# bsxfun/pffdtd

Measured on AMD Instinct MI355X. Metric: Gvoxel-updates/s, higher is better.
Workload: dtype f32; 1 GPU; shoebox 1024^3 7-pt Cartesian fp32, Mb=11 freq-dependent walls (BASELINE.json configs[3]); Nb=12423680, Nbl=6205736, Nba=6254648, numerics=cpu-exact, parallelism=1 GPU, air_variant=0

## Files before the change

include/pffdtd_hip.h:

```cpp
#ifndef PFFDTD_HIP_H
#define PFFDTD_HIP_H

#include <stdint.h>
#include <stddef.h>

#ifdef __cplusplus
extern "C" {
#endif

#define PF_MMB 12
#define PF_MNM 64

typedef struct pf_matquad_f32 { float  b, bd, bDh, bFh; } pf_matquad_f32;
typedef struct pf_matquad_f64 { double b, bd, bDh, bFh; } pf_matquad_f64;

typedef struct pf_simdata {
   int64_t  *bn_ixyz;
   int64_t  *bnl_ixyz;
   int64_t  *bna_ixyz;
   int8_t   *Q_bna;
   int64_t  *in_ixyz;
   int64_t  *out_ixyz;
   int64_t  *out_reorder;
   uint16_t *adj_bn;
   void     *ssaf_bnl;
   uint8_t  *bn_mask;
   int8_t   *mat_bnl;
   int8_t   *K_bn;
   double   *in_sigs;
   double   *u_out;
   int64_t   Ns, Nr, Nt, Npts, Nx, Ny, Nz, Nb, Nbl, Nba;
   double    l, l2;
   int8_t    fcc_flag;
   int8_t    NN;
   int8_t    Nm;
   int8_t   *Mb;
   void     *mat_quads;
   void     *mat_beta;
   double    infac;
   double    sl2, lo2, a2, a1;
   int32_t   real_bytes;
} pf_simdata;

typedef enum pf_status {
   PF_OK = 0,
   PF_ERR_ARG = 1,
   PF_ERR_HIP = 2,
   PF_ERR_NODEV = 3,
   PF_ERR_STATE = 4
} pf_status;

#define PF_NUM_CPU_EXACT       0
#define PF_NUM_GPU_SAFEGUARDED 2

typedef struct pf_opts {
   int32_t device;
   int32_t numerics;
   int32_t slab_first;
   int32_t slab_last;
   int32_t readout_chunk;
   int32_t air_variant;
   int32_t air_chunk;
   int32_t timing;
   void   *ext_u0;
   void   *ext_u1;
   int32_t x_global0;
   int32_t layout;
   int32_t energy;
   int32_t multi_flags;
   int32_t transport;
   int32_t verify_exchange;
   int32_t only_slab;
   double  wall_scale;
} pf_opts;

#define PF_LAYOUT_AUTO      0
#define PF_LAYOUT_EXCHANGED 1
#define PF_LAYOUT_FILE      2

#define PF_TRANSPORT_AUTO 0
#define PF_TRANSPORT_PEER 1
#define PF_TRANSPORT_RCCL 2
#define PF_TRANSPORT_HOST 3

#define PF_MULTI_EVEN_SPLIT  1
#define PF_MULTI_ONE_THREAD  2
#define PF_MULTI_NO_PAIRS    4
#define PF_MULTI_FORCE_PAIRS 8
#define PF_MULTI_CUT_Z      16
#define PF_MULTI_CUT_X      32
#define PF_MULTI_MEASURE_WEIGHTS 128
#define PF_MULTI_NO_TRIPLES 64

typedef struct pf_timing {
   double  air_ms_total;
   int64_t air_launches;
   double  step_ms_total;
   int64_t steps;
   double  tb2_ms_total;
   int64_t tb2_launches;
   int64_t tb2_cells;
   double  tune_ms[3];
   int64_t air_path;
   int64_t tb2_lw;
   int64_t tb2_dirty_tiles;
   int64_t place_candidates;
   double  place_ms[3];
   int64_t wall_blocks[2];
   int64_t tb_steps_per_pass;
   int64_t wall_bricks;
   int64_t wall_three_steps;
   int64_t wall_profile;
} pf_timing;

typedef struct pf_engine pf_engine;

const char *pf_last_error(void);
const char *pf_version(void);
int         pf_device_count(void);
size_t      pf_grid_bytes(int64_t Nx, int64_t Ny, int64_t Nz, int32_t real_bytes);
int64_t     pf_grid_pitch(int64_t Nz, int32_t real_bytes);
void        pf_opts_default(pf_opts *o);

double      pf_run_sim(pf_simdata *sd);
double      pf_run_sim_devices(pf_simdata *sd, int32_t nslabs, const int32_t *devices, const pf_opts *base);
int         pf_slab_partition(const pf_simdata *sd, int32_t nslabs, int32_t even_split, int64_t *cuts);
int         pf_slab_partition_w(const pf_simdata *sd, int32_t nslabs, int32_t even_split, double wall_scale, int64_t *cuts);
int         pf_slab_partition_axis(const pf_simdata *sd, int32_t nslabs, int32_t even_split, double wall_scale, int32_t along_z, int64_t *cuts);
double      pf_slab_wall_scale(pf_simdata *sd, int32_t nslabs, int32_t device, const pf_opts *base);

typedef struct pf_multi pf_multi;
typedef struct pf_multi_info {
   int32_t nslabs;
   int32_t transport;
   int32_t rccl_self;
   int32_t exchange_verified;
   int64_t exchanges_checked;
   int32_t exchange_nonzero;
   int32_t cut_along_z;
   int64_t plane_bytes;
   double  last_run_seconds;
   char    transport_name[64];
   char    transport_note[256];
   double  wall_scale;
   int32_t wall_measured;
} pf_multi_info;
int  pf_multi_create(pf_simdata *sd, int32_t nslabs, const int32_t *devices, const pf_opts *base, pf_multi **out);
int  pf_multi_run(pf_multi *m, int64_t n0, int64_t nsteps);
int  pf_multi_get_info(pf_multi *m, pf_multi_info *info);
int  pf_multi_get_slab(pf_multi *m, int32_t g, int64_t *x0, int64_t *x1, int32_t *device, int32_t *paired, pf_engine **engine);
void pf_multi_destroy(pf_multi *m);

typedef struct pf_rccl_comm pf_rccl_comm;
int  pf_rccl_unique_id(void *id128);
int  pf_rccl_comm_create(const void *id128, int32_t nranks, int32_t rank, int32_t device, pf_rccl_comm **out);
int  pf_rccl_exchange(pf_rccl_comm *c, pf_engine *e, int32_t peer_lo, int32_t peer_hi);
void pf_rccl_comm_destroy(pf_rccl_comm *c);

int  pf_engine_create(const pf_simdata *sd, const pf_opts *opts, pf_engine **out);
void pf_engine_destroy(pf_engine *e);
int  pf_engine_run(pf_engine *e, int64_t n0, int64_t nsteps);
int  pf_engine_step_begin(pf_engine *e, int64_t n);
int  pf_engine_halo_ptrs(pf_engine *e, void **send_lo, void **send_hi, void **recv_lo, void **recv_hi,
                         size_t *plane_bytes);
int  pf_engine_step_end(pf_engine *e, int64_t n);
int  pf_engine_set_spares(pf_engine *e, void *grid2, void *grid3);
int  pf_engine_place_grids(pf_engine *e, void *const *pool, int32_t n, int32_t idx[4]);
int  pf_engine_place_grids5(pf_engine *e, void *const *pool, int32_t n, int32_t idx[5]);
int  pf_engine_state_grids(pf_engine *e, void **u_prev, void **u_cur);
int  pf_engine_layout(pf_engine *e, int64_t *dims, int64_t *pitch, int32_t *exchanged);
void *pf_engine_stream(pf_engine *e, int32_t which);
int  pf_engine_sync(pf_engine *e);
int  pf_engine_flush_outputs(pf_engine *e);
int  pf_engine_get_grid(pf_engine *e, int32_t which, void *host);
int  pf_engine_set_grid(pf_engine *e, int32_t which, const void *host);
int  pf_engine_timing(pf_engine *e, pf_timing *t, int32_t reset);
int  pf_engine_set_timing(pf_engine *e, int32_t on);

int  pf_engine_energy_cfg(pf_engine *e, double h, double c, double Ts, const double *DEF);
int  pf_engine_run_energy(pf_engine *e, int64_t n0, int64_t nsteps, double *H_tot, double *E_lost, double *E_in);

#ifdef __cplusplus
}
#endif
#endif
```

pffdtd_amd/csrc/pf_debug.h:

```cpp
#pragma once
#include "pffdtd_hip.h"
struct pf_opts_x : pf_opts {
   int32_t debug;
   int32_t test_drop_exchange;
   int32_t test_faults;
};
extern "C" void pf_internal_hooks(int32_t debug, int32_t test_drop_exchange, int32_t test_faults);
pf_opts_x pf__take_hooks(const pf_opts *o);
int pf__engine_create_x(const pf_simdata *sd, const pf_opts_x *o, pf_engine **out);
enum : int {
   PF_DBG_RUNTIME_NODES = 0x20,
   PF_DBG_LW32 = 0x100,
   PF_DBG_LW16 = 0x200,
   PF_DBG_LW64 = 0x400,
   PF_DBG_SRC_TILES_SINGLE = 0x40,
   PF_DBG_EDGE_SEPARATE = 0x80,
   PF_DBG_RUNTIME_GEOMETRY = 0x800,
   PF_DBG_SWZ_ON = 0x1000,
   PF_DBG_SWZ_OFF = 0x2000,
   PF_DBG_SINGLE_STEPS = 0x4000,
   PF_DBG_NO_AUTOTUNE = 0x8000,
   PF_DBG_WALLS_BESIDE_BOX = 0x10000,
   PF_DBG_NO_TRIPLES = 0x20000,
   PF_DBG_FCC_PAIR_R4 = 0x40000,
   PF_DBG_THIRD_STEP_LISTS = 0x80000,
   PF_DBG_BND_PLAIN_ORDER = 0x100000,
   PF_DBG_BND_FETCH_ALL = 0x200000,
   PF_DBG_FRAME_GENERIC = 0x400000,
   PF_DBG_GRAPH = 0x800000,
   PF_DBG_XY_TWO_PLUS_ONE = 0x1000000,
   PF_DBG_STRIPS_SPLIT = 0x2000000,
   PF_DBG_WALLS_ONE_STREAM = 0x4000000,
   PF_DBG_WALLS_ALL_GENERIC = 0x8000000,
   PF_DBG_NO_WALL_REGIONS = 0x10000000,
   PF_DBG_BND_ALL_NODES = 0x20000000,
   PF_DBG_STRIPS_TWO_PLUS_ONE = 0x40000000,
};
```

pffdtd_amd/csrc/pf_engine_class.inc:

```
#include <hip/hip_runtime.h>
#include <algorithm>
#include <chrono>
#include <cmath>
#include <cstdarg>
#include <cstdio>
#include <cstring>
#include <mutex>
#include <new>
#include <numeric>
#include <string>
#include <vector>

#include "pffdtd_hip.h"
#include "pf_debug.h"
#include "pf_kernels.h"
#include "pf_air_fused.h"
#include "pf_energy.h"
#include "pf_tb2.h"
#include "pf_tb3.h"
#include "pf_wall.h"
#include "pf_brick.h"

extern "C" void pf__set_error(const char *msg);
extern "C" const char *pf_last_error(void);
extern "C" int pf__axis_exchange_pays(const pf_simdata *sd, int64_t *counts);
extern std::mutex pf__tune_mu[64];

namespace pfeng {
struct EngineBase {
   virtual ~EngineBase() {}
   virtual int run(int64_t n0, int64_t nsteps) = 0;
   virtual int step_begin(int64_t n) = 0;
   virtual int step_end(int64_t n) = 0;
   virtual int halo_ptrs(void **slo, void **shi, void **rlo, void **rhi, size_t *bytes) = 0;
   virtual int state_grids(void **up, void **uc) = 0;
   virtual int layout(int64_t *dims, int64_t *pitch, int32_t *exchanged) = 0;
   virtual int sync() = 0;
   virtual int flush() = 0;
   virtual int set_spares(void *g2, void *g3) = 0;
   virtual int place_grids(void *const *grids, int n, int32_t *idx) = 0;
   virtual int place_grids5(void *const *grids, int n, int32_t *idx) = 0;
   virtual int get_grid(int which, void *host) = 0;
   virtual int set_grid(int which, const void *host) = 0;
   virtual int timing(pf_timing *t, int reset) = 0;
   virtual int set_timing(int on) = 0;
   virtual void *stream(int which) = 0;
   virtual int energy_cfg(double h, double c, double Ts, const double *DEF) = 0;
   virtual int run_energy(int64_t n0, int64_t nsteps, double *H, double *El, double *Ei) = 0;
};
}

namespace {
using pfeng::EngineBase;

int set_err(int code, const char *fmt, ...) {
   char buf[1024];
   va_list ap;
   va_start(ap, fmt);
   vsnprintf(buf, sizeof buf, fmt, ap);
   va_end(ap);
   pf__set_error(buf);
   return code;
}

}

namespace {

#define HIPCHK(expr)                                                                                          \
   do {                                                                                                       \
      hipError_t _e = (expr);                                                                                 \
      if (_e != hipSuccess)                                                                                   \
         return set_err(PF_ERR_HIP, "HIP error %s at %s:%d: %s", hipGetErrorName(_e), __FILE__, __LINE__,     \
                        hipGetErrorString(_e));                                                               \
   } while (0)

#define HIPCHK_V(expr) do { (void)(expr); } while (0)

inline int64_t round_up(int64_t a, int64_t m) { return (a + m - 1) / m * m; }
inline int64_t cdiv(int64_t a, int64_t b) { return (a + b - 1) / b; }

int64_t grid_pitch(int64_t Nz, int32_t real_bytes) { return round_up(Nz, 128 / real_bytes); }

int dpp_ok_cached = -1;
int check_dpp(hipStream_t s) {
   if (dpp_ok_cached >= 0) return dpp_ok_cached;
   int *d = nullptr, h = 0;
   if (hipMalloc(&d, sizeof(int)) != hipSuccess) return 0;
   hipLaunchKernelGGL(pf::k_dpp_selftest, dim3(1), dim3(64), 0, s, d);
   hipMemcpyAsync(&h, d, sizeof(int), hipMemcpyDeviceToHost, s);
   hipStreamSynchronize(s);
   hipFree(d);
   dpp_ok_cached = h;
   return h;
}

struct Range { int64_t b, e; };


template <typename Real> struct Engine : EngineBase {
   pf_simdata sd{};
   pf_opts_x op{};
   int64_t Nx = 0, Ny = 0, Nz = 0, P = 0, plane = 0, npad = 0;
   bool swz = false;
   int64_t fNx = 0, fNy = 0, fNz = 0;
   int64_t Nb = 0, Nbl = 0, Nba = 0, Ns = 0, Nr = 0, Nt = 0;
   int mb_max = 0;
   bool fcc = false, fold = false;
   bool use_dpp = true;
   Real a1, a2, sl2, lo2, l;
   Real *u0 = nullptr, *u1 = nullptr;
   bool own_grids = true;
   std::vector<float> place_ms;
   bool tb2_probe = false;
   std::vector<Real *> own_list;
   uint8_t *mask = nullptr;
   Real *v1_dst = nullptr;
   int lw_force = 0;
   int order_force = -1;
   float tune_ms[3] = {0, 0, 0};
   float pair_margin = 0.99f;
   bool lean = false, need_fold_row = false;
   bool vg = false;
   bool abck = false;
   int vbase = 0;
   bool sg = false;
   int lean_nzt = 0;
   int64_t *d_bn = nullptr, *d_bnl = nullptr, *d_bna = nullptr, *d_in = nullptr, *d_out = nullptr;
   uint16_t *d_adj = nullptr;
   int32_t *d_lossy = nullptr;
   bool fuse_boundary = false;
   int8_t *d_Q = nullptr, *d_mat = nullptr, *d_Mb = nullptr;
   Real *d_ssaf = nullptr, *d_beta = nullptr, *d_insig = nullptr;
   pf::MatQuadT<Real> *d_mq = nullptr;
   Real *ub[3] = {nullptr, nullptr, nullptr};
   Real *u2ba = nullptr, *vh1 = nullptr, *gh1 = nullptr;
   Real *ring = nullptr;
   Real *h_ring = nullptr;
   int64_t ring_depth = 0, ring_fill = 0, ring_n0 = 0;
   std::vector<int64_t> out_row;
   Range bn_lo, bn_mid, bn_hi, bnl_lo, bnl_mid, bnl_hi, bna_lo, bna_mid, bna_hi, in_lo, in_mid, in_hi;
   Range bn_lo2, bn_mid2, bn_hi2, bnl_lo2, bnl_mid2, bnl_hi2, in_lo2, in_mid2, in_hi2;
   Range bn_lo3, bn_mid3, bn_hi3, bnl_lo3, bnl_mid3, bnl_hi3, in_lo3, in_mid3, in_hi3;
   hipStream_t s_main = nullptr, s_edge = nullptr, s_wall = nullptr, s_wall2 = nullptr;
   hipEvent_t ev_pre = nullptr, ev_edge = nullptr, ev_main = nullptr, ev_wall0 = nullptr, ev_wall = nullptr, ev_wall2 = nullptr;
   hipEvent_t ev_src0 = nullptr, ev_src1 = nullptr;
   bool wall_pending = false;
   bool in_step = false;
   bool state_touched = false;
   int64_t steps_done = 0;
   bool graph_ok = false;
   hipGraphExec_t gexec = nullptr;
   int64_t rot_count = 0, g_rot0 = -1;
   int64_t *d_ctr = nullptr;
   bool tb2 = false;
   bool tb2_geom = false, tb2_slab = false;
   int pair_phase = 0;
   bool pair_now = false;
   bool triple_now = false;
   Real *pA = nullptr, *pB = nullptr;
   Real *bufC = nullptr, *bufD = nullptr;
   bool tb3 = false;
   bool tb3_geom = false, tb3_slab = false;
   bool triples() const { return tb3 || tb3_slab; }
   Real *bufE = nullptr;
   Real *home[5] = {nullptr, nullptr, nullptr, nullptr, nullptr};
   static constexpr int tb3_wt = 8, tb3_r = 3, tb3_rows = tb3_wt * tb3_r - 4;
   int tbx0 = 0, tbx1 = 0, tby0 = 0, tby1 = 0, tbz0 = 0, tbz1 = 0;
   int tbzu0 = 0, tbzu1 = 0;
   int szl = 0, szr = 0;
   int tb2_chunk = 16;
   std::vector<std::pair<int, int>> tb_xr;
   int tb_lw = 64, tb_chunk = 16, tb_nxc = 0, tb_nyt = 0, tb_nzt = 0;
   int32_t *tb_clean = nullptr, *tb_dirty = nullptr;
   int32_t *tb_sample = nullptr;
   int64_t tb_nsample = 0;
   double tb_sample_frac = 1.0;
   int64_t tb_nclean = 0, tb_ndirty = 0, tb_clean_cells = 0;
   int32_t *tb_srct = nullptr;
   int64_t tb_nsrct = 0;
   bool src_in_kernel() const { return tb_nsrct > 0; }
   Range src_range() const { return Range{0, src_in_kernel() ? 0 : Ns}; }
   bool tb_order_band = false;
   int32_t *sh_tiles = nullptr;
   static constexpr int fcc_wt = 8;
   int64_t sh_ntiles = 0;
   int sh_nyt = 0, sh_nzt = 0;
   const Real *u0_src = nullptr;
   int lean_yt0 = 0, lean_nyt = -1;
   int lean_x2_begin = 0, lean_x2_end = 0;
   uint32_t *zs_map = nullptr;
   uint16_t *zs_adj = nullptr;
   int32_t *zs_li = nullptr;
   int32_t *zs_rest = nullptr;
   int64_t zs_nrest = 0;
   int zs_mode = 0;
   int32_t *zs_fd = nullptr;
   int64_t zs_nfd = 0;
   const int32_t *bnd_sel = nullptr;
   bool wl_on = false;
   int32_t *edge_sel3 = nullptr; int64_t n_edge_sel3 = 0; bool edge_sel3_failed = false;
   Real *wsT2 = nullptr, *wsT3 = nullptr;
   bool ws_five = false, ws_all3 = false;
   Real *wsP[3] = {nullptr, nullptr, nullptr};
   struct WlGroup { int nreg = 0; pf::WallRegion reg[pf::WALL_MAXREG]; uint32_t blk0[3] = {0, 0, 0}, nblk[3] = {0, 0, 0};
                    uint32_t blk0b = 0, nblkb = 0; int32_t mchunk2[pf::WALL_MAXREG] = {0, 0, 0, 0, 0, 0}; };
   WlGroup wl_grp[4];
   uint4 *wl_blk = nullptr;
   uint4 *wl_pen = nullptr;
   uint32_t *wl_rec = nullptr;
   int32_t *wl_rest = nullptr;
   int64_t wl_nrest = 0;
   pf::Brick *wl_brk = nullptr;
   uint32_t *wl_binfo = nullptr;
   uint2 *wl_blos = nullptr;
   int64_t wl_nbrk = 0, wl_nbown_dbg = 0;
   bool wl_xw[2] = {false, false};
   bool wl_ns3 = false, wl_ns3z = false, wl_no_ns3 = false;
   Real *ubx[2] = {nullptr, nullptr};
   int wl_geo[4] = {0, 0, 0, 0};
   int wl_prof[4] = {0, 0, 0, 0};
   int wl_chunk_want[2] = {0, 0};
   size_t wl_brk_lds = 0;
   Real *vh1b = nullptr, *gh1b = nullptr;
   Real *bs_vout = nullptr, *bs_gout = nullptr;
   Real *Lu = nullptr, *vh_old = nullptr, *u2in = nullptr;
   double *d_acc = nullptr, *d_DEF = nullptr;
   double en_h = 0, en_c = 0, en_Ts = 0;
   bool en_ready = false;
   std::vector<std::pair<hipEvent_t, hipEvent_t>> air_ev, step_ev, tb2_ev, ev_pool;
   pf_timing tm{};

   ~Engine() override { destroy(); }

   void destroy() {
      if (s_main) hipStreamSynchronize(s_main);
      if (s_edge) hipStreamSynchronize(s_edge);
      auto F = [](void *p) { if (p) hipFree(p); };
      for (Real *g : own_list) F(g);
      own_list.clear();
      F(wl_pen); F(wl_rec); F(wl_rest); F(wl_blk); F(wl_brk); F(wl_binfo); F(wl_blos); F(ubx[0]); F(ubx[1]); F(edge_sel3); F(vh1b); F(gh1b); F(d_lossy); F(mask); F(zs_map); F(zs_adj); F(zs_li); F(zs_rest); F(zs_fd); F(tb_clean); F(tb_dirty); F(tb_srct); F(tb_sample); F(sh_tiles); F(Lu); F(vh_old); F(u2in); F(d_acc); F(d_DEF); F(d_bn); F(d_bnl); F(d_bna); F(d_in); F(d_out); F(d_adj); F(d_Q); F(d_mat); F(d_Mb); F(d_ssaf);
      F(d_beta); F(d_insig); F(d_mq); F(ub[0]); F(ub[1]); F(ub[2]); F(u2ba); F(vh1); F(gh1); F(ring);
      if (h_ring) hipHostFree(h_ring);
      for (auto &p : air_ev) { hipEventDestroy(p.first); hipEventDestroy(p.second); }
      for (auto &p : step_ev) { hipEventDestroy(p.first); hipEventDestroy(p.second); }
      for (auto &p : tb2_ev) { hipEventDestroy(p.first); hipEventDestroy(p.second); }
      for (auto &p : ev_pool) { hipEventDestroy(p.first); hipEventDestroy(p.second); }
      if (ev_pre) hipEventDestroy(ev_pre);
      if (ev_edge) hipEventDestroy(ev_edge);
      if (ev_main) hipEventDestroy(ev_main);
      if (ev_src0) hipEventDestroy(ev_src0);
      if (ev_src1) hipEventDestroy(ev_src1);
      ev_src0 = ev_src1 = nullptr;
      if (gexec) hipGraphExecDestroy(gexec);
      if (d_ctr) hipFree(d_ctr);
      if (s_wall) hipStreamDestroy(s_wall);
      if (s_wall2) hipStreamDestroy(s_wall2);
      if (ev_wall0) hipEventDestroy(ev_wall0);
      if (ev_wall) hipEventDestroy(ev_wall);
      if (ev_wall2) hipEventDestroy(ev_wall2);
      if (s_main) hipStreamDestroy(s_main);
      if (s_edge) hipStreamDestroy(s_edge);
      u0 = u1 = nullptr; s_main = s_edge = s_wall = s_wall2 = nullptr; ev_wall0 = ev_wall = ev_wall2 = nullptr;
   }

   inline void decode(int64_t ii, int64_t &ix, int64_t &iy, int64_t &iz) const {
      const int64_t fz = ii % fNz, fy = (ii / fNz) % fNy, fx = ii / (fNz * fNy);
      ix = swz ? fz : fx; iy = fy; iz = swz ? fx : fz;
   }
   inline int64_t pad_idx(int64_t ii) const {
      int64_t ix, iy, iz;
      decode(ii, ix, iy, iz);
      return (ix * Ny + iy) * P + iz;
   }

   template <typename T> int upload(T **dst, const T *src, int64_t n) {
      *dst = nullptr;
      HIPCHK(hipMalloc((void **)dst, std::max<int64_t>(n, 1) * sizeof(T)));
      if (n > 0) HIPCHK(hipMemcpy(*dst, src, n * sizeof(T), hipMemcpyHostToDevice));
      return PF_OK;
   }
   template <typename T> int dzalloc(T **dst, int64_t n) {
      *dst = nullptr;
      size_t bytes = std::max<int64_t>(n, 1) * sizeof(T);
      {
         const hipError_t e = hipMalloc((void **)dst, bytes);
         if (e != hipSuccess) {
            size_t fr = 0, tot = 0;
            (void)hipGetLastError();
            if (hipMemGetInfo(&fr, &tot) != hipSuccess) { fr = tot = 0; (void)hipGetLastError(); }
            return set_err(PF_ERR_HIP, "HIP error %s allocating %zu bytes of engine state (%zu of %zu bytes free on device %d): %s", hipGetErrorName(e), bytes, fr, tot, op.device, hipGetErrorString(e));
         }
      }
      HIPCHK(hipMemset(*dst, 0, bytes));
      return PF_OK;
   }

   template <typename T> T *try_dzalloc(int64_t n) {
      T *p = nullptr;
      const size_t bytes = std::max<int64_t>(n, 1) * sizeof(T);
      if (hipMalloc((void **)&p, bytes) != hipSuccess) { (void)hipGetLastError(); return nullptr; }
      if (hipMemset(p, 0, bytes) != hipSuccess) { (void)hipGetLastError(); hipFree(p); return nullptr; }
      return p;
   }
   void plane_ranges(const std::vector<int64_t> &idx, Range &lo, Range &mid, Range &hi, int w = 1) const {
      const int64_t n = (int64_t)idx.size();
      auto first_ge = [&](int64_t px) { return (int64_t)(std::lower_bound(idx.begin(), idx.end(), px * plane) - idx.begin()); };
      if (w >= 2 && Nx < 4 * w) { lo = mid = hi = {0, 0}; return; }
      const int64_t b1 = first_ge(1), b2 = first_ge(1 + w), b3 = first_ge(Nx - 1 - w), b4 = first_ge(Nx - 1);
      lo = {b1, std::min(b2, b4)};
      if (Nx - 2 > 1) { mid = {b2, std::max(b2, b3)}; hi = {std::max(b2, b3), b4}; }
      else { mid = {b2, b2}; hi = {b2, b2}; }
      (void)n;
   }

   bool fused_ok() const {
      if (!use_dpp) return false;
      if (Nx < 5 || Ny < 5 || Nz < 5) return false;
      if (plane >= ((int64_t)1 << 31)) return false;
      for (int64_t i = 0; i < Nb; i++) {
         int64_t ix, iy, iz;
         decode(sd.bn_ixyz[i], ix, iy, iz);
         if ((op.slab_first && ix == 1) || (op.slab_last && ix == Nx - 2) || iy == 1 || iz == 1 || iz == Nz - 2) return false;
         if (!fold && iy == Ny - 2) return false;
      }
      for (int64_t i = 0; i < Nr; i++) {
         int64_t ix, iy, iz;
         decode(sd.out_ixyz[i], ix, iy, iz);
         if (ix < 1 || iy < 1 || iz < 1 || ix > Nx - 2 || iy > Ny - 2 || iz > Nz - 2) return false;
      }
      int64_t Nyf = fold ? 2 * (Ny - 1) : Ny;
      int64_t expect = 2 * (Nx * Nyf + Nx * Nz + Nyf * Nz) - 12 * (Nx + Nyf + Nz) + 56;
      if (fcc) expect /= 2;
      if (!(op.slab_first && op.slab_last)) return Nba <= expect;
      return Nba == expect;
   }
   bool rigid_separable() const {
      if (!fold) return true;
      for (int64_t i = 0; i < Nb; i++)
         if ((sd.bn_ixyz[i] / fNz) % fNy == fNy - 2) return false;
      return true;
   }

   int decide_swap() {
      swz = false;
      const bool single = op.slab_first && op.slab_last, ext = op.ext_u0 && op.ext_u1;
      const int vb = op.air_variant & 255;
      if (op.debug & 0x1000) {
         if (op.energy) return set_err(PF_ERR_ARG, "debug 0x1000 (axes exchanged in storage): no energy diagnostic");
         swz = true;
         return PF_OK;
      }
      if ((op.debug & 0x2000) || !single || ext || op.energy || vb == 41) return PF_OK;
      int64_t counts[2];
      swz = pf__axis_exchange_pays(&sd, counts) != 0;
      if (counts[0] + counts[1] > 0 && getenv("PFFDTD_VERBOSE") && atoi(getenv("PFFDTD_VERBOSE")) > 0)
         fprintf(stderr, "pffdtd_hip: %ld of %ld boundary nodes have their successor along file x, %ld along file z: storage %s\n", (long)counts[0],
                 (long)sd.Nb, (long)counts[1], swz ? "with the x and z axes exchanged (unit stride along file x)" : "in file order");
      return PF_OK;
   }

   int init(const pf_simdata *s, const pf_opts_x *o) {
      sd = *s;
      op = *o;
      fNx = sd.Nx; fNy = sd.Ny; fNz = sd.Nz;
      Nx = sd.Nx; Ny = sd.Ny; Nz = sd.Nz;
      Nb = sd.Nb; Nbl = sd.Nbl; Nba = sd.Nba; Ns = sd.Ns; Nr = sd.Nr; Nt = sd.Nt;
      if (Nx < 3 || Ny < 3 || Nz < 3) return set_err(PF_ERR_ARG, "grid must be at least 3x3x3 (got %ld %ld %ld)", (long)Nx, (long)Ny, (long)Nz);
      if (sd.Npts != Nx * Ny * Nz) return set_err(PF_ERR_ARG, "Npts != Nx*Ny*Nz");
      if (sd.fcc_flag < 0 || sd.fcc_flag > 2) return set_err(PF_ERR_ARG, "fcc_flag must be 0, 1 or 2");
      if (sd.NN != (sd.fcc_flag ? 12 : 6)) return set_err(PF_ERR_ARG, "NN does not match fcc_flag");
      if (sd.Nm > PF_MNM) return set_err(PF_ERR_ARG, "too many materials (MNm=%d)", PF_MNM);
      if (Nt < 0 || Ns < 0 || Nr < 0 || Nb < 0 || Nbl < 0 || Nba < 0) return set_err(PF_ERR_ARG, "negative count");
      for (int k = 0; k < sd.Nm; k++)
         if (sd.Mb[k] < 0 || sd.Mb[k] > PF_MMB) return set_err(PF_ERR_ARG, "Mb[%d] out of range (MMb=%d)", k, PF_MMB);
      for (int k = 0; k < sd.Nm; k++) mb_max = std::max(mb_max, (int)sd.Mb[k]);
      fcc = sd.fcc_flag > 0;
      fold = sd.fcc_flag == 2;
      a1 = (Real)sd.a1; a2 = (Real)sd.a2; sl2 = (Real)sd.sl2; lo2 = (Real)sd.lo2; l = (Real)sd.l;
      { int rc = decide_swap(); if (rc) return rc; }
      if (swz) std::swap(Nx, Nz);
      P = grid_pitch(Nz, sizeof(Real));
      plane = Ny * P;
      npad = Nx * plane;

      int ndev = 0;
      if (hipGetDeviceCount(&ndev) != hipSuccess || ndev <= 0) return set_err(PF_ERR_NODEV, "no HIP device visible");
      if (op.device < 0 || op.device >= ndev) return set_err(PF_ERR_ARG, "device %d out of range (%d visible)", op.device, ndev);
      HIPCHK(hipSetDevice(op.device));
      int lo_prio = 0, hi_prio = 0;
      hipDeviceGetStreamPriorityRange(&lo_prio, &hi_prio);
      HIPCHK(hipStreamCreateWithPriority(&s_main, hipStreamNonBlocking, lo_prio));
      HIPCHK(hipStreamCreateWithPriority(&s_edge, hipStreamNonBlocking, hi_prio));
      HIPCHK(hipEventCreateWithFlags(&ev_pre, hipEventDisableTiming));
      HIPCHK(hipEventCreateWithFlags(&ev_edge, hipEventDisableTiming));
      HIPCHK(hipEventCreateWithFlags(&ev_main, hipEventDisableTiming));
      HIPCHK(hipEventCreateWithFlags(&ev_src0, hipEventDisableTiming));
      HIPCHK(hipEventCreateWithFlags(&ev_src1, hipEventDisableTiming));
      use_dpp = check_dpp(s_main) == 1;
      if (!use_dpp) return set_err(PF_ERR_HIP, "DPP wave-shift self-test failed on device %d: this library is built for gfx950 (wave64, row_shr / row_shl with bank masks)", op.device);

      if (op.ext_u0 && op.ext_u1) {
         u0 = (Real *)op.ext_u0; u1 = (Real *)op.ext_u1; own_grids = false;
      } else {
         int rc;
         if ((rc = dzalloc(&u0, npad))) return rc;
         if ((rc = dzalloc(&u1, npad))) return rc;
         own_list.push_back(u0); own_list.push_back(u1);
      }

      auto sorted_perm = [&](const int64_t *src, int64_t n, std::vector<int64_t> &idx) {
         std::vector<int64_t> perm(n), key(n);
         std::iota(perm.begin(), perm.end(), 0);
         for (int64_t i = 0; i < n; i++) key[i] = pad_idx(src[i]);
         bool is_sorted = true;
         for (int64_t i = 1; i < n && is_sorted; i++) is_sorted = key[i - 1] <= key[i];
         if (!is_sorted) std::stable_sort(perm.begin(), perm.end(), [&](int64_t a, int64_t b) { return key[a] < key[b]; });
         idx.resize(n);
         for (int64_t i = 0; i < n; i++) idx[i] = key[perm[i]];
         return perm;
      };
      auto in_interior = [&](const int64_t *src, int64_t n, const char *what) -> int {
         for (int64_t i = 0; i < n; i++) {
            const int64_t ii = src[i];
            if (ii < 0 || ii >= sd.Npts) return set_err(PF_ERR_ARG, "%s[%ld]=%ld outside the grid", what, (long)i, (long)ii);
            int64_t ix, iy, iz;
            decode(ii, ix, iy, iz);
            if (ix < 1 || iy < 1 || iz < 1 || ix > Nx - 2 || iy > Ny - 2 || iz > Nz - 2)
               return set_err(PF_ERR_ARG, "%s[%ld]=%ld is not an interior node", what, (long)i, (long)ii);
         }
         return PF_OK;
      };
      int rc;
      if ((rc = in_interior(sd.bn_ixyz, Nb, "bn_ixyz"))) return rc;
      if ((rc = in_interior(sd.bnl_ixyz, Nbl, "bnl_ixyz"))) return rc;
      if ((rc = in_interior(sd.bna_ixyz, Nba, "bna_ixyz"))) return rc;
      if ((rc = in_interior(sd.in_ixyz, Ns, "in_ixyz"))) return rc;
      for (int64_t i = 0; i < Nr; i++)
         if (sd.out_ixyz[i] < 0 || sd.out_ixyz[i] >= sd.Npts) return set_err(PF_ERR_ARG, "out_ixyz[%ld] outside the grid", (long)i);

      std::vector<int64_t> idx;
      {
         auto perm = sorted_perm(sd.bn_ixyz, Nb, idx);
         std::vector<uint16_t> adj(Nb);
         for (int64_t i = 0; i < Nb; i++) adj[i] = sd.adj_bn[perm[i]];
         if ((rc = upload(&d_bn, idx.data(), Nb))) return rc;
         if ((rc = upload(&d_adj, adj.data(), Nb))) return rc;
         plane_ranges(idx, bn_lo, bn_mid, bn_hi);
         plane_ranges(idx, bn_lo2, bn_mid2, bn_hi2, 2);
         plane_ranges(idx, bn_lo3, bn_mid3, bn_hi3, 3);
         vbase = op.air_variant & 255;
         if (op.air_variant & ~(255 | 256)) return set_err(PF_ERR_ARG, "air_variant %d: unknown flag bits", op.air_variant);
         if (vbase != 0 && vbase != 3 && vbase != 4 && vbase != 7 && vbase != 25 && vbase != 40 && vbase != 41)
            return set_err(PF_ERR_ARG, "air_variant %d: choose 0 (auto), 3 (unfused reference sequence), 4 / 7 (barrier-free kernel: virtual ghosts / "
                                       "in-kernel ABC), 25 (lean fused kernel, 7-point), 40 / 41 (blocked pairs); the other variants were retired", op.air_variant);
         if (op.numerics != PF_NUM_CPU_EXACT && op.numerics != PF_NUM_GPU_SAFEGUARDED)
            return set_err(PF_ERR_ARG, "numerics must be PF_NUM_CPU_EXACT (0) or PF_NUM_GPU_SAFEGUARDED (2)");
         sg = op.numerics == PF_NUM_GPU_SAFEGUARDED;
         if (sg && !use_dpp) return set_err(PF_ERR_ARG, "the safeguarded numerics run on the DPP builds of the kernels only");
         const bool ok = fused_ok();
         const int64_t Wseg = 64 * pf::VecOf<Real>::V;
         const bool wide = (double)P / (double)(cdiv(P, Wseg) * Wseg) >= 0.8;
         if (op.energy) { if (vbase != 0 && vbase != 3) return set_err(PF_ERR_ARG, "the energy diagnostic runs the unfused kernel sequence (air_variant 0 or 3)"); }
         else if (vbase == 0 || vbase == 40 || vbase == 41) {
            if ((vbase == 40 || vbase == 41) && !ok) return set_err(PF_ERR_ARG, "air_variant %d (blocked pairs) requested but the fused-path preconditions do not hold", op.air_variant);
            lean = ok && !fcc && (wide || vbase != 0);
            abck = ok && fcc;
            vg = ok && !lean && !fcc;
         }
         else if (vbase == 7) { abck = true; if (!ok) return set_err(PF_ERR_ARG, "air_variant 7 (in-kernel ABC) requested but its preconditions do not hold"); }
         else if (vbase == 4) { vg = true; if (!ok) return set_err(PF_ERR_ARG, "air_variant 4 (virtual ghost shell) requested but its preconditions do not hold"); }
         else if (vbase == 25) {
            lean = true;
            if (fcc) return set_err(PF_ERR_ARG, "air_variant 25 (lean fused kernel) is 7-point Cartesian only");
            if (!ok) return set_err(PF_ERR_ARG, "air_variant 25 (lean fused kernel) requested but its preconditions do not hold");
         }
         need_fold_row = fold && !rigid_separable();
         HIPCHK(hipDeviceSynchronize());
         lean_nzt = (int)cdiv(P, 64 * pf::VecOf<Real>::V);
         if ((rc = dzalloc(&mask, npad / 8))) return rc;
         HIPCHK(hipDeviceSynchronize());
         hipLaunchKernelGGL(pf::k_mask_init, dim3((unsigned)cdiv(Nx * Ny * (P / 16), 256)), dim3(256), 0, s_main, mask, Nx, Ny, P, Nz,
                            sd.fcc_flag == 1 ? 1 + (op.x_global0 & 1) : 0);
         if (Nb) hipLaunchKernelGGL(pf::k_mask_set, dim3((unsigned)cdiv(Nb, 256)), dim3(256), 0, s_main, mask, d_bn, Nb);
         HIPCHK(hipGetLastError());
      }
      {
         auto perm = sorted_perm(sd.bnl_ixyz, Nbl, idx);
         std::vector<Real> ssaf(Nbl);
         std::vector<int8_t> mat(Nbl);
         for (int64_t i = 0; i < Nbl; i++) {
            ssaf[i] = ((const Real *)sd.ssaf_bnl)[perm[i]];
            mat[i] = sd.mat_bnl[perm[i]];
            if (mat[i] < 0 || mat[i] >= sd.Nm) return set_err(PF_ERR_ARG, "mat_bnl[%ld]=%d out of range", (long)perm[i], mat[i]);
         }
         if ((rc = upload(&d_bnl, idx.data(), Nbl))) return rc;
         if ((rc = upload(&d_ssaf, ssaf.data(), Nbl))) return rc;
         if ((rc = upload(&d_mat, mat.data(), Nbl))) return rc;
         plane_ranges(idx, bnl_lo, bnl_mid, bnl_hi);
         plane_ranges(idx, bnl_lo2, bnl_mid2, bnl_hi2, 2);
         plane_ranges(idx, bnl_lo3, bnl_mid3, bnl_hi3, 3);
         for (int i = 0; i < 3; i++) if ((rc = dzalloc(&ub[i], Nbl))) return rc;
         if ((rc = dzalloc(&vh1, round_up(Nbl, 64) * PF_MMB))) return rc;
         if ((rc = dzalloc(&gh1, round_up(Nbl, 64) * PF_MMB))) return rc;
         const int64_t nm = std::max<int64_t>(sd.Nm, 1);
         if ((rc = upload(&d_mq, (const pf::MatQuadT<Real> *)sd.mat_quads, sd.Nm ? nm * PF_MMB : 0))) return rc;
         if ((rc = upload(&d_beta, (const Real *)sd.mat_beta, sd.Nm))) return rc;
         if ((rc = upload(&d_Mb, sd.Mb, sd.Nm))) return rc;
      }
      {
         std::vector<int64_t> hb(Nb), hl(Nbl);
         if (Nb) HIPCHK(hipMemcpy(hb.data(), d_bn, Nb * sizeof(int64_t), hipMemcpyDeviceToHost));
         if (Nbl) HIPCHK(hipMemcpy(hl.data(), d_bnl, Nbl * sizeof(int64_t), hipMemcpyDeviceToHost));
         std::vector<int32_t> lz(Nb, -1);
         int64_t j = 0;
         bool subset = Nbl < ((int64_t)1 << 31);
         for (int64_t i = 0; i < Nb && j < Nbl; i++) {
            if (hb[i] == hl[j]) {
               if (j + 1 < Nbl && hl[j + 1] == hl[j]) { subset = false; break; }
               lz[i] = (int32_t)j++;
            } else if (hb[i] > hl[j]) { subset = false; break; }
         }
         if (j != Nbl) subset = false;
         for (int64_t i = 1; i < Nb && subset; i++) if (hb[i] == hb[i - 1]) subset = false;
         fuse_boundary = subset && Nb > 0 && !(op.air_variant & 256) && !op.energy;
         if (fuse_boundary) { if ((rc = upload(&d_lossy, lz.data(), Nb))) return rc; }
      }
      {
         auto perm = sorted_perm(sd.bna_ixyz, Nba, idx);
         std::vector<int8_t> Q(Nba);
         for (int64_t i = 0; i < Nba; i++) Q[i] = sd.Q_bna[perm[i]];
         if ((rc = upload(&d_bna, idx.data(), Nba))) return rc;
         if ((rc = upload(&d_Q, Q.data(), Nba))) return rc;
         if ((rc = dzalloc(&u2ba, Nba))) return rc;
         plane_ranges(idx, bna_lo, bna_mid, bna_hi);
      }
      {
         auto perm = sorted_perm(sd.in_ixyz, Ns, idx);
         std::vector<Real> sig((size_t)std::max<int64_t>(Ns * Nt, 1));
         for (int64_t i = 0; i < Ns; i++)
            for (int64_t n = 0; n < Nt; n++) sig[i * Nt + n] = (Real)sd.in_sigs[perm[i] * Nt + n];
         if ((rc = upload(&d_in, idx.data(), Ns))) return rc;
         if ((rc = upload(&d_insig, sig.data(), Ns * Nt))) return rc;
         plane_ranges(idx, in_lo, in_mid, in_hi);
         plane_ranges(idx, in_lo2, in_mid2, in_hi2, 2);
         plane_ranges(idx, in_lo3, in_mid3, in_hi3, 3);
      }
      {
         auto perm = sorted_perm(sd.out_ixyz, Nr, idx);
         out_row = perm;
         if ((rc = upload(&d_out, idx.data(), Nr))) return rc;
         ring_depth = op.readout_chunk > 0 ? op.readout_chunk : 1024;
         if (Nt > 0) ring_depth = std::min<int64_t>(ring_depth, Nt);
         ring_depth = std::max<int64_t>(ring_depth, 1);
         if ((rc = dzalloc(&ring, Nr * ring_depth))) return rc;
         HIPCHK(hipHostMalloc((void **)&h_ring, std::max<int64_t>(Nr * ring_depth, 1) * sizeof(Real), hipHostMallocDefault));
      }
      std::lock_guard<std::mutex> tune_lock(pf__tune_mu[op.device & 63]);
      { int rc = init_tb2(); if (rc) return rc; }
      tb2_probe = true;
      pair_margin = 1.12f;
      { int rc = autotune(); if (rc) { tb2_probe = false; return rc; } }
      { int rc = sample_placement(); if (rc) { tb2_probe = false; return rc; } }
      pair_margin = 0.99f;
      if (tb2) { int rc = autotune(); if (rc) { tb2_probe = false; return rc; } }
      else if (fcc) { int rc = autotune_fcc_lw(); if (rc) { tb2_probe = false; return rc; } }
      tb2_probe = false;
      if (tb3) tb3_remember_home();
      if (!tb2 && op.slab_first && op.slab_last) { int rc = sample_placement_single(); if (rc) return rc; }
      graph_ok = (op.debug & 0x800000) && op.slab_first && op.slab_last && !tb2 && !op.timing && !op.energy;
      if (getenv("PFFDTD_VERBOSE") && atoi(getenv("PFFDTD_VERBOSE")) > 0)
         fprintf(stderr, "pffdtd_hip: engine on device %d, %ldx%ldx%ld %s %s, interior path: %s%s, numerics: %s, %d-lane row segments\n", op.device, (long)Nx, (long)Ny, (long)Nz,
                 fcc ? "13-point" : "7-point", sizeof(Real) == 4 ? "fp32" : "fp64",
                 tb3 ? ((wl_ns3 && wl_ns3z) ? "three steps per pass (k_tb3), the shell too: three-step wall regions + bricks" :
                        wl_ns3 ? "three steps per pass (k_tb3), shell: three-step x / y regions + bricks, column strips two steps + one" :
                        wl_nbrk ? "three steps per pass (k_tb3), shell: wall regions two steps + one, frame as bricks" :
                                  "three steps per pass (k_tb3), shell as wall regions + one single step") : tb2 ? "temporally blocked pairs" : (lean ? "lean fused kernel" : (vg ? "barrier-free kernel, virtual ghosts" : (abck ? "barrier-free kernel, in-kernel ABC" : "unfused reference sequence"))),
                 tb2_geom && !tb2 ? " (pairs when the caller hands over four grids)" : (swz ? " (stored with the file's x and z axes exchanged)" : ""), sg ? "GPU-safeguarded" : "CPU-exact", tb2 ? tb_lw : (lean ? 64 : pick_lw()));
      HIPCHK(hipDeviceSynchronize());
      return PF_OK;
   }

#include "pf_engine_blocking.inc"
#include "pf_engine_walls.inc"
#include "pf_engine_blocked_steps.inc"
#include "pf_engine_tune.inc"
#include "pf_engine_launch.inc"
   int build_graph() {
      if (!d_ctr) HIPCHK(hipMalloc((void **)&d_ctr, 2 * sizeof(int64_t)));
      hipGraph_t g = nullptr;
      HIPCHK(hipStreamBeginCapture(s_main, hipStreamCaptureModeThreadLocal));
      for (int k = 0; k < 6; k++) {
         fold_x0 = 0; fold_x1 = (int)Nx;
         launch_pre(s_main);
         launch_air(s_main, 1, (int)Nx - 1);
         launch_abc(s_main, {0, Nba});
         launch_rigid(s_main, {0, Nb});
         launch_fd(s_main, {0, Nbl});
         launch_io(s_main, 0, true, {0, Ns}, d_ctr);
         hipLaunchKernelGGL(pf::k_ctr_tick, dim3(1), dim3(1), 0, s_main, d_ctr);
         rotate();
      }
      rot_count -= 6;
      const hipError_t e = hipStreamEndCapture(s_main, &g);
      if (e != hipSuccess || !g) { graph_ok = false; (void)hipGetLastError(); return PF_OK; }
      if (hipGraphInstantiate(&gexec, g, nullptr, nullptr, 0) != hipSuccess) { gexec = nullptr; graph_ok = false; (void)hipGetLastError(); }
      hipGraphDestroy(g);
      g_rot0 = ((rot_count % 6) + 6) % 6;
      return PF_OK;
   }
   int step_six(int64_t n) {
      hipLaunchKernelGGL(pf::k_ctr_set, dim3(1), dim3(1), 0, s_main, d_ctr, n, ring_fill);
      HIPCHK(hipGraphLaunch(gexec, s_main));
      for (int k = 0; k < 6; k++) rotate();
      if (ring_fill == 0) ring_n0 = n;
      ring_fill += 6;
      steps_done += 6;
      if (ring_fill == ring_depth) return flush();
      return PF_OK;
   }
   void rotate() {
      std::swap(u0, u1);
      Real *t = ub[2]; ub[2] = ub[1]; ub[1] = ub[0]; ub[0] = t;
      rot_count++;
   }
   int after_step(int64_t n) {
      if (ring_fill == 0) ring_n0 = n;
      ring_fill++;
      steps_done++;
      if (ring_fill == ring_depth) return flush();
      return PF_OK;
   }

   int step_single(int64_t n) {
      if (n < 0 || n >= Nt) return set_err(PF_ERR_ARG, "step %ld outside [0,Nt=%ld)", (long)n, (long)Nt);
      std::pair<hipEvent_t, hipEvent_t> ev{};
      if (op.timing) {
         if (!ev_pool.empty()) { ev = ev_pool.back(); ev_pool.pop_back(); }
         else { hipEventCreate(&ev.first); hipEventCreate(&ev.second); }
         hipEventRecord(ev.first, s_main);
      }
      fold_x0 = 0; fold_x1 = (int)Nx;
      launch_pre(s_main);
      launch_air(s_main, 1, (int)Nx - 1);
      launch_abc(s_main, {0, Nba});
      launch_rigid(s_main, {0, Nb});
      launch_fd(s_main, {0, Nbl});
      launch_io(s_main, n, true, {0, Ns});
      if (op.timing) { hipEventRecord(ev.second, s_main); step_ev.push_back(ev); }
      HIPCHK(hipGetLastError());
      rotate();
      return after_step(n);
   }

   int energy_cfg(double h, double c, double Ts, const double *DEF) override {
      if (!op.energy) return set_err(PF_ERR_STATE, "engine was not created with pf_opts.energy=1");
      if (sd.fcc_flag == 2) return set_err(PF_ERR_ARG, "the energy diagnostic is defined for fcc_flag 0 and 1 (as in the reference)");
      HIPCHK(hipSetDevice(op.device));
      en_h = h; en_c = c; en_Ts = Ts;
      int rc;
      if (!Lu) {
         if ((rc = dzalloc(&Lu, npad))) return rc;
         if ((rc = dzalloc(&vh_old, round_up(Nbl, 64) * PF_MMB))) return rc;
         if ((rc = dzalloc(&u2in, Ns))) return rc;
         if ((rc = dzalloc(&d_acc, (int64_t)pf::EN_NACC))) return rc;
         if ((rc = upload(&d_DEF, DEF, (int64_t)std::max<int>(sd.Nm, 1) * PF_MMB * 3))) return rc;
      }
      HIPCHK(hipDeviceSynchronize());
      en_ready = true;
      return PF_OK;
   }
   int run_energy(int64_t n0, int64_t nsteps, double *H, double *El, double *Ei) override {
      if (!en_ready) return set_err(PF_ERR_STATE, "call pf_engine_energy_cfg first");
      if (in_step) return set_err(PF_ERR_STATE, "pf_engine_run_energy inside a split-phase step");
      HIPCHK(hipSetDevice(op.device));
      hipStream_t s = s_main;
      const double V = fcc ? 2.0 : 1.0, l2d = sd.l2, ld = sd.l;
      const dim3 g3((unsigned)cdiv(Nz, 256), (unsigned)(Ny - 2), (unsigned)(Nx - 2));
      auto g1 = [](int64_t n, int b) { return dim3((unsigned)std::max<int64_t>(cdiv(n, b), 1)); };
      for (int64_t n = n0; n < n0 + nsteps; n++) {
         if (n < 0 || n >= Nt) return set_err(PF_ERR_ARG, "step %ld outside [0,Nt=%ld)", (long)n, (long)Nt);
         double acc[pf::EN_NACC];
         HIPCHK(hipMemsetAsync(d_acc, 0, sizeof(double) * pf::EN_NACC, s));
         hipLaunchKernelGGL(pf::k_energy_int<Real>, g3, dim3(256), 0, s, u1, u0, Lu, Nx, Ny, Nz, P, plane, l2d, d_acc);
         if (Nba) hipLaunchKernelGGL(pf::k_energy_abc<Real>, g1(Nba, 256), dim3(256), 0, s, u1, u0, Lu, d_bna, d_Q, Nba, l2d, d_acc);
         if (Nbl) hipLaunchKernelGGL(pf::k_energy_stored<Real>, g1(Nbl, 256), dim3(256), 0, s, vh1, gh1, d_ssaf, d_mat, d_Mb, d_DEF, Nbl, en_Ts, d_acc);
         if (Ns) hipLaunchKernelGGL(pf::k_energy_in<Real>, g1(Ns, 64), dim3(64), 0, s, u0, u2in, d_in, d_insig, Ns, Nt, n, 0, d_acc);
         if (Nbl) HIPCHK(hipMemcpyAsync(vh_old, vh1, sizeof(Real) * round_up(Nbl, 64) * PF_MMB, hipMemcpyDeviceToDevice, s));
         fold_x0 = 0; fold_x1 = (int)Nx;
         launch_pre(s);
         if (fcc) {
            hipLaunchKernelGGL((pf::k_lap_air<Real, true>), g3, dim3(256), 0, s, u1, Lu, mask, Nx, Ny, Nz, P, plane);
            if (Nb) hipLaunchKernelGGL((pf::k_lap_bn<Real, true>), g1(Nb, 256), dim3(256), 0, s, u1, Lu, d_bn, d_adj, P, plane, Nb);
         } else {
            hipLaunchKernelGGL((pf::k_lap_air<Real, false>), g3, dim3(256), 0, s, u1, Lu, mask, Nx, Ny, Nz, P, plane);
            if (Nb) hipLaunchKernelGGL((pf::k_lap_bn<Real, false>), g1(Nb, 256), dim3(256), 0, s, u1, Lu, d_bn, d_adj, P, plane, Nb);
         }
         launch_air(s, 1, (int)Nx - 1);
         launch_abc(s, {0, Nba});
         launch_rigid(s, {0, Nb});
         launch_fd(s, {0, Nbl});
         launch_io(s, n, true, {0, Ns});
         if (Nbl) hipLaunchKernelGGL(pf::k_energy_loss<Real>, g1(Nbl, 256), dim3(256), 0, s, vh_old, vh1, d_ssaf, d_mat, d_Mb, d_DEF, Nbl, d_acc);
         if (Nba) hipLaunchKernelGGL(pf::k_energy_abcloss<Real>, g1(Nba, 256), dim3(256), 0, s, u0, u2ba, d_bna, d_Q, Nba, d_acc);
         if (Ns) hipLaunchKernelGGL(pf::k_energy_in<Real>, g1(Ns, 64), dim3(64), 0, s, u0, u2in, d_in, d_insig, Ns, Nt, n, 1, d_acc);
         HIPCHK(hipGetLastError());
         HIPCHK(hipMemcpyAsync(acc, d_acc, sizeof(acc), hipMemcpyDeviceToHost, s));
         HIPCHK(hipStreamSynchronize(s));
         H[n] = V * 0.5 * en_h * acc[pf::EN_INT] - V * 0.5 * en_h * acc[pf::EN_ABC] + V * 0.5 * en_c / l2d * acc[pf::EN_STORED];
         El[n + 1] = El[n] + V * 0.25 * en_h / ld * acc[pf::EN_LOSS] + 0.5 * V * en_h / ld * acc[pf::EN_ABCLOSS];
         Ei[n + 1] = Ei[n] + (V * en_h / l2d) * 0.5 * acc[pf::EN_IN];
         rotate();
         int rc = after_step(n);
         if (rc) return rc;
      }
      return flush();
   }

   int run(int64_t n0, int64_t nsteps) override {
      if (in_step || pair_phase) return set_err(PF_ERR_STATE, "pf_engine_run inside a split-phase step (pair)");
      HIPCHK(hipSetDevice(op.device));
      for (int64_t n = n0; n < n0 + nsteps;) {
         int rc;
         if (tb3) tb3_pick();
         if (tb3 && n + 3 <= n0 + nsteps && ring_fill + 3 <= ring_depth) {
            if ((rc = step_triple(n))) return rc;
            n += 3;
         } else if (tb3 && n + 2 <= n0 + nsteps && ring_fill + 2 <= ring_depth) {
            if ((rc = step_pair(n))) return rc;
            n += 2;
         } else if (tb2 && !tb3 && n + 4 <= n0 + nsteps && ring_fill + 4 <= ring_depth) {
            if ((rc = step_pair(n))) return rc;
            if ((rc = step_pair(n + 2))) return rc;
            n += 4;
         } else if (graph_ok && n + 6 <= n0 + nsteps && ring_fill + 6 <= ring_depth && (gexec || g_rot0 < 0) &&
                    (g_rot0 < 0 || ((rot_count % 6) + 6) % 6 == g_rot0)) {
            if (!gexec) { if ((rc = build_graph())) return rc; if (!gexec) continue; }
            if ((rc = step_six(n))) return rc;
            n += 6;
         } else {
            if ((rc = step_single(n))) return rc;
            n++;
         }
         if (op.timing && air_ev.size() >= 512) { rc = harvest(); if (rc) return rc; }
      }
      int rc = flush();
      if (rc) return rc;
      return harvest();
   }

#include "pf_engine_slab_steps.inc"
   int sync() override {
      HIPCHK(hipSetDevice(op.device));
      HIPCHK(hipStreamSynchronize(s_edge));
      HIPCHK(hipStreamSynchronize(s_main));
      return PF_OK;
   }

   int flush() override {
      if (ring_fill == 0) return PF_OK;
      HIPCHK(hipSetDevice(op.device));
      HIPCHK(hipStreamSynchronize(s_edge));
      if (Nr > 0) {
         HIPCHK(hipMemcpyAsync(h_ring, ring, (size_t)(Nr * ring_depth) * sizeof(Real), hipMemcpyDeviceToHost, s_main));
      }
      HIPCHK(hipStreamSynchronize(s_main));
      if (sd.u_out)
         for (int64_t t = 0; t < Nr; t++) {
            double *dst = sd.u_out + out_row[t] * Nt + ring_n0;
            const Real *src = h_ring + t * ring_depth;
            for (int64_t k = 0; k < ring_fill; k++) dst[k] = (double)src[k];
         }
      ring_fill = 0;
      return PF_OK;
   }

   int harvest() {
      if (!op.timing) return PF_OK;
      HIPCHK(hipStreamSynchronize(s_edge));
      HIPCHK(hipStreamSynchronize(s_main));
      for (auto &p : air_ev) {
         float ms = 0;
         HIPCHK(hipEventElapsedTime(&ms, p.first, p.second));
         tm.air_ms_total += ms; tm.air_launches++;
         ev_pool.push_back(p);
      }
      air_ev.clear();
      for (auto &p : tb2_ev) {
         float ms = 0;
         HIPCHK(hipEventElapsedTime(&ms, p.first, p.second));
         tm.tb2_ms_total += ms; tm.tb2_launches += 1;
         ev_pool.push_back(p);
      }
      tb2_ev.clear();
      tm.tb2_cells = tb_clean_cells;
      tm.tb_steps_per_pass = triples() ? 3 : ((tb2 || tb2_slab) ? 2 : 0);
      for (auto &p : step_ev) {
         float ms = 0;
         HIPCHK(hipEventElapsedTime(&ms, p.first, p.second));
         tm.step_ms_total += ms; tm.steps++;
         ev_pool.push_back(p);
      }
      step_ev.clear();
      return PF_OK;
   }
   int timing(pf_timing *t, int reset) override {
      int rc = harvest();
      if (rc) return rc;
      for (int i = 0; i < 3; i++) tm.tune_ms[i] = tune_ms[i];
      tm.air_path = (tb2 || tb2_slab) ? 2 : (lean ? 0 : (vg ? 1 : -1));
      tm.tb2_lw = (tb2 || tb2_slab) ? tb_lw : 0;
      tm.tb2_dirty_tiles = (tb2 || tb2_slab) ? tb_ndirty : 0;
      tm.place_candidates = (int64_t)place_ms.size();
      if (!place_ms.empty()) {
         tm.place_ms[0] = place_ms[0];
         tm.place_ms[1] = *std::min_element(place_ms.begin(), place_ms.end());
         tm.place_ms[2] = *std::max_element(place_ms.begin(), place_ms.end());
      }
      tm.wall_blocks[0] = tm.wall_blocks[1] = 0;
      if (wl_on)
         for (const WlGroup &g : wl_grp) { tm.wall_blocks[0] += g.nblk[0] + g.nblk[2]; tm.wall_blocks[1] += g.nblk[1]; }
      tm.wall_bricks = wl_on ? wl_nbrk : 0;
      tm.wall_three_steps = (wl_on && (tb3 || (tb3_slab && ws_all3))) ? ((wl_ns3 ? 1 : 0) | (wl_ns3z ? 8 : 0) | (wl_xw[0] ? 0x10 : 0) | (wl_xw[1] ? 0x20 : 0)) : 0;
      tm.wall_profile = (((tm.wall_three_steps & 1) && wl_geo[0] == 6 && wl_prof[0]) ? 1 : 0) | (((tm.wall_three_steps & 8) && wl_geo[3] == 16 && wl_prof[3]) ? 8 : 0);
      if (t) *t = tm;
      if (reset) tm = pf_timing{};
      return PF_OK;
   }

   int set_timing(int on) override {
      if (in_step) return set_err(PF_ERR_STATE, "pf_engine_set_timing inside a step");
      int rc = harvest();
      if (rc) return rc;
      op.timing = on ? 1 : 0;
      return PF_OK;
   }
   int get_grid(int which, void *host) override {
      HIPCHK(hipSetDevice(op.device));
      int rc = sync();
      if (rc) return rc;
      const Real *src = which == 0 ? (pair_phase > 0 ? (const Real *)u0_src : (const Real *)u0) : u1;
      if ((lean || vg) && which == 1) {
         launch_flips(s_main);
         HIPCHK(hipStreamSynchronize(s_main));
      }
      if (swz) {
         Real *tmp = nullptr;
         HIPCHK(hipMalloc((void **)&tmp, (size_t)sd.Npts * sizeof(Real)));
         hipLaunchKernelGGL((pf::k_storage_to_file<Real>), dim3((unsigned)cdiv(sd.Npts, 256)), dim3(256), 0, s_main, src, tmp, fNx, fNy, fNz, Ny, P);
         const hipError_t e = hipMemcpyAsync(host, tmp, (size_t)sd.Npts * sizeof(Real), hipMemcpyDeviceToHost, s_main);
         hipStreamSynchronize(s_main);
         hipFree(tmp);
         HIPCHK(e);
         return PF_OK;
      }
      HIPCHK(hipMemcpy2D(host, Nz * sizeof(Real), src, P * sizeof(Real), Nz * sizeof(Real), Nx * Ny, hipMemcpyDeviceToHost));
      return PF_OK;
   }
   int set_grid(int which, const void *host) override {
      HIPCHK(hipSetDevice(op.device));
      int rc = sync();
      if (rc) return rc;
      Real *dst = which == 0 ? u0 : u1;
      state_touched = true;
      if (swz) {
         Real *tmp = nullptr;
         HIPCHK(hipMalloc((void **)&tmp, (size_t)sd.Npts * sizeof(Real)));
         hipError_t e = hipMemcpyAsync(tmp, host, (size_t)sd.Npts * sizeof(Real), hipMemcpyHostToDevice, s_main);
         hipLaunchKernelGGL((pf::k_file_to_storage<Real>), dim3((unsigned)cdiv(sd.Npts, 256)), dim3(256), 0, s_main, tmp, dst, fNx, fNy, fNz, Ny, P);
         hipStreamSynchronize(s_main);
         hipFree(tmp);
         HIPCHK(e);
         return PF_OK;
      }
      HIPCHK(hipMemcpy2D(dst, P * sizeof(Real), host, Nz * sizeof(Real), Nz * sizeof(Real), Nx * Ny, hipMemcpyHostToDevice));
      return PF_OK;
   }
   void *stream(int which) override { return which == 1 ? (void *)s_edge : (void *)s_main; }
};

}
```

pffdtd_amd/csrc/pf_engine_walls.inc:

```
   int wl_lo_option(int t0, bool prefer_split) const {
      const bool split_ok = t0 >= 10 && t0 + 2 - 4 <= 16, wide_ok = sizeof(Real) == 4 && t0 + 2 <= 20;
      if (t0 + 2 <= 12) return 1;
      if (split_ok && (prefer_split || !wide_ok)) return 2;
      return wide_ok ? 3 : 0;
   }
   int wl_hi_option(int t1, bool prefer_split) const {
      const int z1 = std::min((t1 - 2) / 4 * 4, (int)P - 12), zw = (int)round_up(Nz - 12, 4), s0 = zw + 4, z2 = (t1 - 2) / 4 * 4;
      const int z20 = std::min((t1 - 2) / 4 * 4, (int)P - 20);
      const bool split_ok = zw >= 0 && zw + 12 <= P && s0 > t1 && s0 + 2 - z2 <= 16 && z2 + 16 <= P && (int)Nz - 1 - zw <= 11;
      const bool wide_ok = sizeof(Real) == 4 && z20 >= 0 && z20 + 20 >= Nz && t1 - z20 >= 2;
      if (z1 >= 0 && z1 + 12 >= Nz && t1 - z1 >= 2) return 1;
      if (split_ok && (prefer_split || !wide_ok)) return 2;
      return wide_ok ? 3 : 0;
   }
   void free_walls() {
      auto F = [](auto *&p) { if (p) hipFree((void *)p); p = nullptr; };
      F(wl_pen); F(wl_rec); F(wl_rest); F(wl_blk); F(wl_brk); F(wl_binfo); F(wl_blos); F(vh1b); F(gh1b); F(ubx[0]); F(ubx[1]);
      wl_nbrk = 0; wl_brk_lds = 0; wl_ns3 = wl_ns3z = false;
      for (int &p : wl_prof) p = 0;
      wl_xw[0] = wl_xw[1] = false;
      wl_on = false;
      for (auto &g : wl_grp) g = WlGroup{};
   }
   int init_walls(bool slab = false) {
      wl_on = false;
      const bool single = op.slab_first && op.slab_last;
      const bool vb = getenv("PFFDTD_VERBOSE") && atoi(getenv("PFFDTD_VERBOSE")) > 1;
#define WL_NO(why) do { if (vb) fprintf(stderr, "pffdtd_hip: no wall regions (%s)\n", why); return PF_OK; } while (0)
      if (slab ? (!tb2_slab || single) : (!tb2 || !single)) WL_NO("not a pair-stepping engine of this kind");
      if (fcc || tb_xr.empty() || swz || (op.debug & 0x10000000)) WL_NO("13-point / no box / exchanged axes / switched off");
      if (Nb > 0 && !fuse_boundary) WL_NO("boundary pass not fused");
      if (Nbl >= ((int64_t)1 << 24) || Nb >= ((int64_t)1 << 31)) WL_NO("too many nodes");
      constexpr int DPS = 8, V = pf::VecOf<Real>::V;
      if (!slab && (tbx0 + 2 > DPS || Nx - tbx1 + 2 > DPS)) WL_NO("x margins");
      if (tby0 + 2 > DPS || Ny - tby1 + 2 > DPS) WL_NO("y margins");
      if ((!slab && Nx < 2 * DPS) || Ny < 2 * DPS) WL_NO("grid too small");
      if (slab && (tbx0 < 3 || tbx1 > Nx - 3 || steps_done > 0)) WL_NO("slab: box reaches the edge planes, or stepping has begun");
      for (int64_t i = 0; i < Ns; i++) {
         int64_t ix, iy, iz;
         decode(sd.in_ixyz[i], ix, iy, iz);
         if ((!slab && (ix < tbx0 + 1 || ix > tbx1 - 2)) || iy < tby0 + 1 || iy > tby1 - 2 || iz < tbz0 + 1 || iz > tbz1 - 2) WL_NO("a source within a cell of the shell");
      }
      std::vector<int64_t> hb(Nb);
      std::vector<uint16_t> hadj(Nb);
      std::vector<int32_t> hl(Nb, -1);
      if (Nb) {
         HIPCHK(hipMemcpy(hb.data(), d_bn, Nb * sizeof(int64_t), hipMemcpyDeviceToHost));
         HIPCHK(hipMemcpy(hadj.data(), d_adj, Nb * sizeof(uint16_t), hipMemcpyDeviceToHost));
         HIPCHK(hipMemcpy(hl.data(), d_lossy, Nb * sizeof(int32_t), hipMemcpyDeviceToHost));
      }
      struct Bar { int a0[3], a1[3], axis, nchunk, first; };
      std::vector<Bar> bars;
      std::vector<pf::Brick> hbrk;
      std::vector<uint32_t> hinfo;
      std::vector<std::vector<uint2>> hlos;
      int blen = 0;
      const int Ng[3] = {(int)Nx, (int)Ny, (int)Nz};
      const bool slab3 = slab && tb3_geom;
      constexpr int DPS3 = 10;
      const bool prefer_split = (op.debug & PF_DBG_STRIPS_SPLIT) != 0 || sizeof(Real) != 4;
      const bool can3 = !wl_no_ns3 && !(op.debug & PF_DBG_XY_TWO_PLUS_ONE) && sizeof(Real) == 4 &&
                        (!op.slab_first || tbx0 + 3 <= DPS3) && (!op.slab_last || (int)Nx - tbx1 + 3 <= DPS3) && Nx >= 2 * DPS3 && tby0 + 3 <= DPS3 && (int)Ny - tby1 + 3 <= DPS3 && Ny >= 2 * DPS3;
      const bool can3z = can3 && !(op.debug & PF_DBG_STRIPS_TWO_PLUS_ONE) && wl_lo_option(tbz0, prefer_split) == 3 && wl_hi_option(tbz1, prefer_split) == 3 && tbz0 + 3 <= 20 &&
                         tbz1 - std::min((tbz1 - 2) / 4 * 4, (int)P - 20) >= 3;
      const bool xlo_shell = op.slab_first != 0, xhi_shell = op.slab_last != 0;
      bool bricks = (!slab || (slab3 && can3 && can3z)) && !(op.debug & (PF_DBG_FRAME_GENERIC | PF_DBG_THIRD_STEP_LISTS | PF_DBG_WALLS_ALL_GENERIC)) && tbzu0 >= 2 && tbzu1 <= (int)Nz - 2 && tbzu1 - tbzu0 >= 8;
      for (int64_t i = 0; i < Ns && bricks; i++) {
         int64_t ix, iy, iz;
         decode(sd.in_ixyz[i], ix, iy, iz);
         if (slab && ((ix < tbx0 - 4 && !xlo_shell) || (ix > tbx1 + 3 && !xhi_shell))) continue;
         if (ix < tbx0 + 2 || ix > tbx1 - 3 || iy < tby0 + 2 || iy > tby1 - 3 || iz < tbz0 + 2 || iz > tbz1 - 3) bricks = false;
      }
      if (bricks) {
         const int X[2][2] = {{1, tbx0}, {tbx1, (int)Nx - 1}}, Y[2][2] = {{1, tby0}, {tby1, (int)Ny - 1}}, Z[2][2] = {{1, tbzu0}, {tbzu1, (int)Nz - 1}};
         auto add = [&](const int *xr, const int *yr, const int *zr, int axis) {
            Bar b{{xr[0], yr[0], zr[0]}, {xr[1], yr[1], zr[1]}, axis, 0, 0};
            if (xr[1] > xr[0] && yr[1] > yr[0] && zr[1] > zr[0]) bars.push_back(b);
         };
         const int ZA[2] = {1, (int)Nz - 1}, YB[2] = {tby0, tby1}, XB[2] = {tbx0, tbx1};
         for (int i = 0; i < 2; i++) {
            if (!(i == 0 ? xlo_shell : xhi_shell)) continue;
            for (int j = 0; j < 2; j++) add(X[i], Y[j], ZA, 2);
            for (int j = 0; j < 2; j++) add(X[i], YB, Z[j], 1);
         }
         for (int i = 0; i < 2; i++) for (int j = 0; j < 2; j++) add(XB, Y[i], Z[j], 0);
         constexpr int H = pf::BRICK_HALO;
         auto ext = [&](int o0, int o1, int d, int &e0, int &e1) { e0 = std::max(o0 - H, 1); e1 = std::min(o1 + H, Ng[d] - 1); };
         bool ok = false;
         for (int L : {16, 8, 4}) {
            blen = L; ok = true;
            hbrk.clear(); hinfo.clear(); hlos.clear();
            for (Bar &b : bars) {
               b.first = (int)hbrk.size();
               b.nchunk = (int)cdiv(b.a1[b.axis] - b.a0[b.axis], L);
               for (int c = 0; c < b.nchunk; c++) {
                  pf::Brick k{};
                  int64_t cells = 1;
                  for (int d = 0; d < 3; d++) {
                     k.o0[d] = d == b.axis ? b.a0[d] + c * L : b.a0[d];
                     k.o1[d] = d == b.axis ? std::min(b.a0[d] + (c + 1) * L, b.a1[d]) : b.a1[d];
                     int e0, e1;
                     ext(k.o0[d], k.o1[d], d, e0, e1);
                     k.e0[d] = e0; k.en[d] = e1 - e0;
                     cells *= k.en[d];
                  }
                  if (pf::brick_lds_bytes<Real>(cells, (int)sd.Nm) > 60 * 1024 || hinfo.size() + (size_t)cells >= ((size_t)1 << 31)) { ok = false; break; }
                  k.info_off = (uint32_t)hinfo.size();
                  for (int ix = 0; ix < k.en[0]; ix++) for (int iy = 0; iy < k.en[1]; iy++) for (int iz = 0; iz < k.en[2]; iz++) {
                     const int g[3] = {k.e0[0] + ix, k.e0[1] + iy, k.e0[2] + iz};
                     uint32_t Q = 0;
                     for (int d = 0; d < 3; d++) Q += ((g[d] == 1 && (d > 0 || xlo_shell)) || (g[d] == Ng[d] - 2 && (d > 0 || xhi_shell))) ? 1u : 0u;
                     hinfo.push_back(Q << 8);
                  }
                  hbrk.push_back(k);
               }
               if (!ok) break;
            }
            if (!ok) continue;
            hlos.assign(hbrk.size(), {});
            for (int64_t nb = 0; nb < Nb && ok; nb++) {
               const int64_t ix = hb[nb] / plane, rem = hb[nb] % plane, iy = rem / P, iz = rem % P;
               const int g[3] = {(int)ix, (int)iy, (int)iz};
               for (const Bar &b : bars) {
                  bool in = true;
                  for (int d = 0; d < 3 && in; d++) in = g[d] >= std::max(b.a0[d] - H, 1) && g[d] < std::min(b.a1[d] + H, Ng[d] - 1);
                  if (!in) continue;
                  const int t = g[b.axis] - b.a0[b.axis];
                  for (int c = std::max((t - H) / L - 1, 0); c <= std::min((t + H) / L + 1, b.nchunk - 1); c++) {
                     pf::Brick &k = hbrk[(size_t)(b.first + c)];
                     if (g[b.axis] < k.e0[b.axis] || g[b.axis] >= k.e0[b.axis] + k.en[b.axis]) continue;
                     if ((g[0] == 1 && xlo_shell) || (g[0] == Ng[0] - 2 && xhi_shell) || g[1] == 1 || g[1] == Ng[1] - 2 || g[2] == 1 || g[2] == Ng[2] - 2) { ok = false; break; }
                     const uint32_t idx = ((uint32_t)(g[0] - k.e0[0]) * (uint32_t)k.en[1] + (uint32_t)(g[1] - k.e0[1])) * (uint32_t)k.en[2] + (uint32_t)(g[2] - k.e0[2]);
                     hinfo[k.info_off + idx] = (uint32_t)(hadj[nb] & 63u) | 0x40u | (hl[nb] >= 0 ? 0x80u : 0u);
                     if (hl[nb] >= 0) {
                        bool own = true;
                        for (int d = 0; d < 3; d++) own = own && g[d] >= k.o0[d] && g[d] < k.o1[d];
                        hlos[(size_t)(b.first + c)].push_back(make_uint2(idx | (own ? 0x80000000u : 0u), (uint32_t)hl[nb]));
                     }
                  }
                  if (!ok) break;
               }
            }
            if (!ok) break;
            for (const auto &v : hlos) if (v.size() > (size_t)pf::BRICK_KN * pf::BRICK_T) ok = false;
            if (ok) break;
         }
         if (!ok || hbrk.empty()) { bricks = false; bars.clear(); hbrk.clear(); hinfo.clear(); hlos.clear(); }
      }
      auto in_frame = [&](int64_t ix, int64_t iy, int64_t iz) {
         const int64_t g[3] = {ix, iy, iz};
         for (const Bar &b : bars) {
            bool in = true;
            for (int d = 0; d < 3 && in; d++) in = g[d] >= b.a0[d] && g[d] < b.a1[d];
            if (in) return true;
         }
         return false;
      };
      std::vector<pf::WallRegion> reg;
      std::vector<int> dps, grp;
      const bool tb3_want = slab ? slab3 : bufE != nullptr;
      const bool ns3 = bricks && tb3_want && can3;
      const int DPX = ns3 ? DPS3 : DPS;
      const bool ns3z = ns3 && can3z;
      auto mk = [&](int group, int mode, int nbase, int kg, int ko0, int ko1, int dp, int l0, int l1, int m0, int m1) {
         pf::WallRegion R{};
         R.mode = mode; R.nbase = nbase; R.kg = kg; R.ko0 = ko0; R.ko1 = ko1;
         const bool h3 = ns3 && (mode != 2 || (ns3z && group == 3));
         R.hl = h3 ? 3 : 2; R.lt = 64 - 2 * R.hl; R.hm = h3 ? 2 : 1;
         R.kb0 = std::max(ko0 - R.hl, 0); R.kb1 = std::min(ko1 + R.hl, dp);
         R.l0 = l0; R.l1 = l1; R.m0 = m0; R.m1 = m1;
         int want = slab ? 4 : 16;
         if (slab && ns3 && (mode != 2 || (ns3z && group == 3))) {
            want = 12;
            if (const char *e = getenv("PFFDTD_SLAB_WALL_CHUNK")) if (atoi(e) > 0) want = atoi(e);
         }
         if (!slab && wl_chunk_want[mode == 2 ? 1 : 0] > 0) want = wl_chunk_want[mode == 2 ? 1 : 0];
         const int len = m1 - m0, nmc = (int)std::max<int64_t>(cdiv(len, want), 1);
         R.mchunk = (int)cdiv(len, nmc);
         R.nlt = (int)cdiv(l1 - l0, R.lt);
         R.nlp = R.nlt * R.lt + 2 * R.hl;
         reg.push_back(R); dps.push_back(dp); grp.push_back(group);
      };
      wl_chunk_want[0] = wl_chunk_want[1] = 0;
      if (!slab && bricks) {
         auto pick = [&](int64_t tiles, int64_t len, int64_t slots) {
            for (int64_t r = 1; r <= 8; r++) {
               const int64_t nmc = std::max<int64_t>(slots * r / std::max<int64_t>(tiles, 1), 1), ch = cdiv(len, nmc);
               if (ch <= 80) return (int)std::max<int64_t>(ch, 4);
            }
            return 16;
         };
         const int64_t lt_xy = 4 * cdiv(tbzu1 - tbzu0, ns3 ? 58 : pf::WALL_LT), lt_z = 2 * cdiv(tby1 - tby0, ns3z ? 58 : pf::WALL_LT);
         wl_chunk_want[0] = pick(lt_xy, std::max(tby1 - tby0, tbx1 - tbx0), (ns3 || sizeof(Real) == 8) ? 1024 : 2048);
         wl_chunk_want[1] = pick(lt_z, tbx1 - tbx0, 1024);
         if (const char *e = getenv("PFFDTD_WALL_CHUNK")) { int a = 0, b = 0; if (sscanf(e, "%d,%d", &a, &b) == 2 && a > 0 && b > 0) { wl_chunk_want[0] = a; wl_chunk_want[1] = b; } }
      }
      const int zl0 = bricks ? tbzu0 : 1, zl1 = bricks ? tbzu1 : (int)Nz - 1, ym0 = bricks ? tby0 : 1, ym1 = bricks ? tby1 : (int)Ny - 1;
      const bool xw0 = slab ? (bricks && xlo_shell) : true, xw1 = slab ? (bricks && xhi_shell) : true;
      if (xw0) mk(0, 0, 0, 0, 1, tbx0, DPX, zl0, zl1, ym0, ym1);
      if (xw1) mk(0, 0, (int)Nx - DPX, DPX - 1, tbx1 - ((int)Nx - DPX), DPX - 1, DPX, zl0, zl1, ym0, ym1);
      mk(0, 1, 0, 0, 1, tby0, DPX, zl0, zl1, tbx0, tbx1);
      mk(0, 1, (int)Ny - DPX, DPX - 1, tby1 - ((int)Ny - DPX), DPX - 1, DPX, zl0, zl1, tbx0, tbx1);
      int zb = 0;
      bool zok = true;
      {
         const int opt = wl_lo_option(tbz0, prefer_split);
         if (opt == 1) mk(1, 2, 0, 0, 1, tbz0, 12, tby0, tby1, tbx0, tbx1);
         else if (opt == 2) {
            mk(1, 2, 0, 0, 1, 8, 12, tby0, tby1, tbx0, tbx1);
            mk(2, 2, 4, -1, 8 - 4, tbz0 - 4, 16, tby0, tby1, tbx0, tbx1);
         } else if (opt == 3) mk(3, 2, 0, 0, 1, tbz0, 20, tby0, tby1, tbx0, tbx1);
         else zok = false;
      }
      {
         const int z1 = std::min((tbz1 - 2) / 4 * 4, (int)P - 12);
         const int zw = (int)round_up(Nz - 12, 4), s0 = zw + 4;
         const int z2 = (tbz1 - 2) / 4 * 4;
         const int z20 = std::min((tbz1 - 2) / 4 * 4, (int)P - 20);
         const int opt = wl_hi_option(tbz1, prefer_split);
         if (opt == 1) { zb = z1; mk(1, 2, z1, (int)Nz - 1 - z1, tbz1 - z1, (int)Nz - 1 - z1, 12, tby0, tby1, tbx0, tbx1); }
         else if (opt == 2) {
            zb = zw;
            mk(1, 2, zw, (int)Nz - 1 - zw, 4, (int)Nz - 1 - zw, 12, tby0, tby1, tbx0, tbx1);
            mk(2, 2, z2, -1, tbz1 - z2, s0 - z2, 16, tby0, tby1, tbx0, tbx1);
         } else if (opt == 3) { zb = z20; mk(3, 2, z20, (int)Nz - 1 - z20, tbz1 - z20, (int)Nz - 1 - z20, 20, tby0, tby1, tbx0, tbx1); }
         else zok = false;
      }
      if (!zok) WL_NO("column strips too wide for the pencils");
#undef WL_NO
      const int nregs = (int)reg.size();
      std::vector<uint32_t> rloc((size_t)nregs);
      {
         int cnt[4] = {0, 0, 0, 0};
         for (int i = 0; i < nregs; i++) {
            if (cnt[grp[i]] >= pf::WALL_MAXREG) return PF_OK;
            rloc[i] = (uint32_t)cnt[grp[i]]++;
         }
      }
      int64_t npen = 0;
      for (int i = 0; i < nregs; i++) { reg[i].pen_off = npen; npen += (int64_t)(reg[i].m1 - reg[i].m0 + 2 * reg[i].hm) * reg[i].nlp; }
      if (npen >= ((int64_t)1 << 31)) return PF_OK;
      auto frame = [&](const pf::WallRegion &R, int64_t ix, int64_t iy, int64_t iz, int &k, int &lc, int &m) {
         if (R.mode == 0) { k = (int)ix - R.nbase; lc = (int)iz; m = (int)iy; }
         else if (R.mode == 1) { k = (int)iy - R.nbase; lc = (int)iz; m = (int)ix; }
         else { k = (int)iz - R.nbase; lc = (int)iy; m = (int)ix; }
      };
      std::vector<int8_t> owner(Nb, 8);
      struct Key { int32_t r, m, lc, k, li; };
      std::vector<Key> keys;
      keys.reserve((size_t)Nbl);
      std::vector<int32_t> rest;
      for (int64_t nb = 0; nb < Nb; nb++) {
         const int64_t ix = hb[nb] / plane, rem = hb[nb] % plane, iy = rem / P, iz = rem % P;
         int r = 8, k = 0, lc = 0, m = 0;
         for (int i = 0; i < nregs; i++) {
            int kk, ll, mm;
            frame(reg[i], ix, iy, iz, kk, ll, mm);
            if (kk >= reg[i].ko0 && kk < reg[i].ko1 && ll >= reg[i].l0 && ll < reg[i].l1 && mm >= reg[i].m0 && mm < reg[i].m1) { r = i; k = kk; lc = ll; m = mm; break; }
         }
         owner[nb] = (int8_t)r;
         const Range &midr = tb3_geom ? bn_mid3 : bn_mid2;
         if (r == 8 && bricks && in_frame(ix, iy, iz)) r = 9;
         owner[nb] = (int8_t)r;
         if (r == 8 && (!slab || (nb >= midr.b && nb < midr.e))) rest.push_back((int32_t)nb);
         if (hl[nb] >= 0) keys.push_back({r, m, lc, k, hl[nb]});
      }
      if ((int64_t)keys.size() != Nbl) return PF_OK;
      std::stable_sort(keys.begin(), keys.end(), [](const Key &a, const Key &b) {
         if (a.r != b.r) return a.r < b.r;
         if (a.r >= 8) return a.li < b.li;
         if (a.m != b.m) return a.m < b.m;
         if (a.lc != b.lc) return a.lc < b.lc;
         return a.k < b.k;
      });
      std::vector<int32_t> newli((size_t)Nbl);
      for (int64_t j = 0; j < Nbl; j++) newli[keys[j].li] = (int32_t)j;
      std::vector<uint4> pen((size_t)npen, make_uint4(0u, 0u, 0u, 0u));
      auto visit = [&](auto &&fn) {
         for (int64_t nb = 0; nb < Nb; nb++) {
            const int64_t ix = hb[nb] / plane, rem = hb[nb] % plane, iy = rem / P, iz = rem % P;
            for (int i = 0; i < nregs; i++) {
               const pf::WallRegion &R = reg[i];
               int k, lc, m;
               frame(R, ix, iy, iz, k, lc, m);
               if (k < std::max(1, R.ko0 - (R.hl - 1)) || k > std::min(dps[i] - 2, R.ko1 + (R.hl - 2)) || lc < R.l0 - (R.hl - 1) || lc > R.l1 + (R.hl - 2) ||
                   m < R.m0 - R.hm || m > R.m1 + R.hm - 1) continue;
               fn(nb, R.pen_off + (int64_t)(m - (R.m0 - R.hm)) * R.nlp + (lc - (R.l0 - R.hl)), k);
            }
         }
      };
      visit([&](int64_t, int64_t pi, int k) { pen[(size_t)pi].x |= 1u << k; });
      int64_t nrec = 0;
      for (int64_t i = 0; i < npen; i++) { pen[(size_t)i].y = (uint32_t)nrec; nrec += __builtin_popcount(pen[(size_t)i].x); }
      if (nrec >= ((int64_t)1 << 27)) return PF_OK;
      std::vector<uint32_t> rec((size_t)std::max<int64_t>(nrec, 1), 0u);
      visit([&](int64_t nb, int64_t pi, int k) {
         uint4 &e = pen[(size_t)pi];
         const uint32_t jn = (uint32_t)__builtin_popcount(e.x & ((1u << k) - 1u));
         const uint32_t adj = (uint32_t)(hadj[nb] & 63u);
         rec[(e.y & 0x7ffffffu) + jn] = adj | (hl[nb] >= 0 ? (0x40u | ((uint32_t)newli[hl[nb]] << 8)) : 0u);
         if (jn < 5) {
            e.z |= adj << (6 * jn);
            if (hl[nb] >= 0) {
               if ((e.w & 31u) == 0u) { e.w |= (uint32_t)newli[hl[nb]] << 8; e.y |= (uint32_t)k << 27; }
               e.w |= 1u << jn;
            }
         }
      });
      int rc;
      free_walls();
      auto no_room = [&]() { free_walls(); (void)hipGetLastError(); pf__set_error(""); if (vb) fprintf(stderr, "pffdtd_hip: no wall regions (no device memory for their tables)\n"); return PF_OK; };
      vh1b = try_dzalloc<Real>(round_up(Nbl, 64) * PF_MMB);
      gh1b = vh1b ? try_dzalloc<Real>(round_up(Nbl, 64) * PF_MMB) : nullptr;
      if (!gh1b) return no_room();
      if ((rc = upload(&wl_pen, pen.data(), npen))) return no_room();
      if ((rc = upload(&wl_rec, rec.data(), nrec))) return no_room();
      wl_nrest = (int64_t)rest.size();
      if ((rc = upload(&wl_rest, rest.data(), wl_nrest))) return no_room();
      if (!slab || slab3) {
         for (int k = 0; k < 2; k++) { ubx[k] = try_dzalloc<Real>(std::max<int64_t>(Nbl, 1)); if (!ubx[k]) return no_room(); }
      }
      if (bricks) {
         std::vector<uint2> flat;
         int64_t nbown = 0;
         size_t lds = 0;
         for (size_t b = 0; b < hbrk.size(); b++) {
            hbrk[b].los_off = (uint32_t)flat.size(); hbrk[b].nlos = (uint32_t)hlos[b].size();
            for (uint2 e : hlos[b]) {
               e.y = (uint32_t)newli[e.y];
               flat.push_back(e);
               if (e.x >> 31) nbown++;
            }
            lds = std::max(lds, pf::brick_lds_bytes<Real>((int64_t)hbrk[b].en[0] * hbrk[b].en[1] * hbrk[b].en[2], (int)sd.Nm));
         }
         if ((rc = upload(&wl_brk, hbrk.data(), (int64_t)hbrk.size()))) return no_room();
         if ((rc = upload(&wl_binfo, hinfo.data(), (int64_t)hinfo.size()))) return no_room();
         if ((rc = upload(&wl_blos, flat.data(), (int64_t)flat.size()))) return no_room();
         wl_nbrk = (int64_t)hbrk.size(); wl_brk_lds = lds; wl_nbown_dbg = nbown;
      }
      if (Nbl) {
         std::vector<int64_t> bl(Nbl), bl2(Nbl);
         std::vector<Real> sf(Nbl), sf2(Nbl);
         std::vector<int8_t> mt(Nbl), mt2(Nbl);
         HIPCHK(hipMemcpy(bl.data(), d_bnl, Nbl * sizeof(int64_t), hipMemcpyDeviceToHost));
         HIPCHK(hipMemcpy(sf.data(), d_ssaf, Nbl * sizeof(Real), hipMemcpyDeviceToHost));
         HIPCHK(hipMemcpy(mt.data(), d_mat, Nbl * sizeof(int8_t), hipMemcpyDeviceToHost));
         for (int64_t j = 0; j < Nbl; j++) { bl2[newli[j]] = bl[j]; sf2[newli[j]] = sf[j]; mt2[newli[j]] = mt[j]; }
         HIPCHK(hipMemcpy(d_bnl, bl2.data(), Nbl * sizeof(int64_t), hipMemcpyHostToDevice));
         HIPCHK(hipMemcpy(d_ssaf, sf2.data(), Nbl * sizeof(Real), hipMemcpyHostToDevice));
         HIPCHK(hipMemcpy(d_mat, mt2.data(), Nbl * sizeof(int8_t), hipMemcpyHostToDevice));
         for (int64_t nb = 0; nb < Nb; nb++) if (hl[nb] >= 0) hl[nb] = newli[hl[nb]];
         HIPCHK(hipMemcpy(d_lossy, hl.data(), Nb * sizeof(int32_t), hipMemcpyHostToDevice));
      }
      for (auto &g : wl_grp) g = WlGroup{};
      for (int i = 0; i < nregs; i++) {
         WlGroup &g = wl_grp[grp[i]];
         g.reg[g.nreg++] = reg[i];
      }
      for (int gi = 0; gi < 4; gi++) {
         const WlGroup &g = wl_grp[gi];
         int gd = 0;
         for (int i = 0; i < g.nreg; i++) {
            const pf::WallRegion &R = g.reg[i];
            const int dp = gi == 0 ? DPX : (gi == 1 ? 12 : (gi == 2 ? 16 : 20));
            const int NNp = R.mode == 2 ? (int)Nz : (R.mode == 1 ? (int)Ny : (int)Nx);
            int d = -1;
            if (R.kg == 0 && R.ko0 == 1 && R.nbase == 0) d = R.ko1;
            else if (R.kg == dp - 1 && R.ko1 == dp - 1 && R.nbase == NNp - dp) d = dp - R.ko0;
            if (d <= 0 || R.hl != 3 || (gd && d != gd)) { gd = -1; break; }
            gd = d;
         }
         wl_geo[gi] = (gd > 0 && !(op.debug & PF_DBG_RUNTIME_GEOMETRY)) ? gd : 0;
      }
      std::vector<uint4> lists[12];
      std::vector<uint4> lists2;
      int64_t nfast = 0, ngen = 0;
      bool second = false;
      auto build = [&](int i, int mchunk) {
         const pf::WallRegion &R = reg[i];
         const int NL = R.mode == 2 ? (int)Ny : (int)Nz, NM = R.mode == 0 ? (int)Ny : (int)Nx;
         const int nmc = (int)cdiv(R.m1 - R.m0, mchunk);
         for (int c = 0; c < nmc; c++)
            for (int jt = 0; jt < R.nlt; jt++) {
               const int ms = R.m0 + c * mchunk, me = std::min(ms + mchunk, R.m1);
               const int lc0 = R.l0 - (R.hl - 1) + R.lt * jt, lc1 = std::min(R.l0 + R.lt * jt + R.lt + (R.hl - 2), R.l1 + (R.hl - 2));
               const int mlo = ms - R.hm, mhi = me + R.hm - 1;
               bool fast = lc0 >= 2 && lc1 <= NL - 3 && mlo >= 2 && mhi <= NM - 3 && !(op.debug & 0x8000000);
               const uint4 ref = pen[(size_t)(R.pen_off + (int64_t)(mlo - (R.m0 - R.hm)) * R.nlp + (lc0 - (R.l0 - R.hl)))];
               if (__builtin_popcount(ref.x) > 5 || __builtin_popcount(ref.w & 31u) > 1) fast = false;
               for (int m = mlo; m <= mhi && fast; m++) {
                  const uint4 *row = pen.data() + (size_t)(R.pen_off + (int64_t)(m - (R.m0 - R.hm)) * R.nlp - (R.l0 - R.hl));
                  for (int lc = lc0; lc <= lc1; lc++) {
                     const uint4 &e = row[lc];
                     if (e.x != ref.x || e.z != ref.z || (e.w & 31u) != (ref.w & 31u) || (e.y >> 27) != (ref.y >> 27)) { fast = false; break; }
                  }
               }
               const uint32_t rl = rloc[i];
               const uint4 b = make_uint4(rl | ((uint32_t)jt << 3) | ((uint32_t)c << 16), ref.x, ref.z, (ref.w & 31u) | ((ref.y >> 27) << 8));
               if (second) { if (fast) lists2.push_back(b); continue; }
               lists[3 * grp[i] + (fast ? (ref.x == 0u && R.mode == 2 ? 2 : 0) : 1)].push_back(b);
               (fast ? nfast : ngen)++;
            }
      };
      for (int i = 0; i < nregs; i++) build(i, reg[i].mchunk);
      wl_grp[0].nblkb = 0;
      if (ns3) {
         second = true;
         for (int i = 0; i < nregs; i++) if (grp[i] == 0) { wl_grp[0].mchunk2[rloc[i]] = std::max(reg[i].mchunk / 2, 4); build(i, wl_grp[0].mchunk2[rloc[i]]); }
         second = false;
      }
      {
         std::vector<uint4> all;
         for (int q = 0; q < 12; q++) { wl_grp[q / 3].blk0[q % 3] = (uint32_t)all.size(); wl_grp[q / 3].nblk[q % 3] = (uint32_t)lists[q].size(); all.insert(all.end(), lists[q].begin(), lists[q].end()); }
         wl_grp[0].blk0b = (uint32_t)all.size(); wl_grp[0].nblkb = (uint32_t)lists2.size(); all.insert(all.end(), lists2.begin(), lists2.end());
         if ((rc = upload(&wl_blk, all.data(), (int64_t)all.size()))) return no_room();
      }
      for (int gi = 0; gi < 4; gi++) {
         wl_prof[gi] = 0;
         const std::vector<uint4> &bl = lists[3 * gi];
         if (sizeof(Real) != 4 || (gi != 0 && gi != 3) || wl_geo[gi] <= 0 || bl.empty() || !lists[3 * gi + 2].empty() || (op.debug & PF_DBG_RUNTIME_NODES)) continue;
         const int dp = gi == 0 ? DPX : 20;
         for (int pr = 1; pr <= pf::WALL_NPROF && !wl_prof[gi]; pr++) {
            bool all = true;
            for (const uint4 &b : bl) {
               const pf::WallRegion &R = wl_grp[gi].reg[b.x & 7u];
               const pf::WallNodes n = pf::wall_profile_words(R.mode, R.kg != 0, dp, pr);
               if (b.y != n.x || b.z != n.z || b.w != n.w) { all = false; break; }
            }
            if (all) wl_prof[gi] = pr;
         }
      }
      wl_ns3 = ns3; wl_ns3z = ns3z;
      if ((ns3 && wl_grp[0].nblk[1] > 0) || (ns3z && wl_grp[3].nblk[1] > 0)) {
         wl_no_ns3 = true;
         return init_walls(slab);
      }
      wl_on = true;
      wl_xw[0] = slab && xw0; wl_xw[1] = slab && xw1;
      if (getenv("PFFDTD_VERBOSE") && atoi(getenv("PFFDTD_VERBOSE")) > 0)
         fprintf(stderr, "pffdtd_hip: wall regions: box x [%d,%d) y [%d,%d) z [%d,%d), %ld pencils, %ld node records, %ld of %ld boundary nodes left to the list kernel, column pencils of %d cells from column %d; %ld blocks alike, %ld generic; frame: %ld bricks of %d cells along their bar (%ld cells with their halos, %ld frequency-dependent nodes owned, %zu bytes of LDS)\n",
                 tbx0, tbx1, tby0, tby1, tbz0, tbz1, (long)npen, (long)nrec, (long)wl_nrest, (long)Nb, dps.back(), zb, (long)nfast, (long)ngen, (long)wl_nbrk, blen, (long)hinfo.size(), (long)wl_nbown_dbg, wl_brk_lds);
      return PF_OK;
   }
   void launch_walls(hipStream_t s, hipStream_t s_gen, const Real *A, const Real *B, Real *C, Real *D, Real *P0, Real *P1, const Real *P2, int ns = 2) {
      launch_walls_x(s, s_gen, A, B, C, D, nullptr, P2, P1, P0, P1, nullptr, ns, 0xf);
   }
   void launch_walls_x(hipStream_t s, hipStream_t s_gen, const Real *A, const Real *B, Real *C, Real *D, Real *E, const Real *x2, const Real *x1, Real *o1, Real *o2, Real *o3,
                       int ns, unsigned gmask) {
      pf::WallParams<Real> wp{};
      wp.A = A; wp.B = B; wp.C = C; wp.D = D; wp.E = E;
      wp.plane = plane; wp.Nx = (int)Nx; wp.Ny = (int)Ny; wp.Nz = (int)Nz; wp.P = (int)P; wp.first = op.slab_first; wp.last = op.slab_last;
      wp.pen = wl_pen; wp.rec = wl_rec;
      wp.sv_in = vh1; wp.sg_in = gh1; wp.sv_out = ns == 1 ? vh1 : vh1b; wp.sg_out = ns == 1 ? gh1 : gh1b;
      wp.x2 = x2; wp.x1 = x1; wp.o1 = o1; wp.o2 = o2; wp.o3 = o3;
      wp.ssaf = d_ssaf; wp.mat = d_mat; wp.Mb = d_Mb; wp.mq = d_mq; wp.beta = d_beta;
      wp.lo2 = lo2; wp.sl2 = sl2; wp.l = l; wp.mmax = mb_max; wp.nmat = sd.Nm;
      for (int gi = 0; gi < 4; gi++) {
         if (!((gmask >> gi) & 1u)) continue;
         const WlGroup &g = wl_grp[gi];
         wp.nreg = g.nreg;
         for (int i = 0; i < g.nreg; i++) wp.reg[i] = g.reg[i];
         for (int q = 0; q < 3; q++) {
            if (!g.nblk[q]) continue;
            wp.blk = wl_blk + g.blk0[q];
            dim3 gd(g.nblk[q]), b(64);
            if (gi == 0 && q == 0 && wl_ns3 && ns == 2 && g.nblkb > 0) {
               wp.blk = wl_blk + g.blk0b; gd = dim3(g.nblkb);
               for (int i = 0; i < g.nreg; i++) wp.reg[i].mchunk = g.mchunk2[i];
            }
            hipStream_t st = q == 1 ? s_gen : s;
#define PF_WALL_N(DP, VEC, S, NSV) do { if (q == 2) { if constexpr (VEC) hipLaunchKernelGGL((pf::k_wall2<Real, DP, VEC, true, false, 12, S, NSV>), gd, b, 0, st, wp, a1, a2); } \
                              else if (mb_max <= 4) { \
                                 if (q == 0) hipLaunchKernelGGL((pf::k_wall2<Real, DP, VEC, true, true, 4, S, NSV>), gd, b, 0, st, wp, a1, a2); \
                                 else hipLaunchKernelGGL((pf::k_wall2<Real, DP, VEC, false, true, 4, S, NSV>), gd, b, 0, st, wp, a1, a2); \
                              } else { \
                                 if (q == 0) hipLaunchKernelGGL((pf::k_wall2<Real, DP, VEC, true, true, 12, S, NSV>), gd, b, 0, st, wp, a1, a2); \
                                 else hipLaunchKernelGGL((pf::k_wall2<Real, DP, VEC, false, true, 12, S, NSV>), gd, b, 0, st, wp, a1, a2); } } while (0)
#define PF_WALL_S(DP, VEC, S) do { if (ns == 1) PF_WALL_N(DP, VEC, S, 1); else PF_WALL_N(DP, VEC, S, 2); } while (0)
#define PF_WALL(DP, VEC) do { if (sg) PF_WALL_S(DP, VEC, true); else PF_WALL_S(DP, VEC, false); } while (0)
#define PF_WALL3_N(S, NSV, GDV, PRV, MCLO) do { if (q != 0) break; \
                              if (mb_max <= 4 || MCLO) hipLaunchKernelGGL((pf::k_wall2<Real, 10, false, true, true, 4, S, NSV, GDV, PRV>), gd, b, 0, st, wp, a1, a2); \
                              else hipLaunchKernelGGL((pf::k_wall2<Real, 10, false, true, true, MCLO ? 4 : 12, S, NSV, GDV, PRV>), gd, b, 0, st, wp, a1, a2); } while (0)
#define PF_WALL3P(NSV, GDV, PRV, MCLO) do { if (sg) PF_WALL3_N(true, NSV, GDV, PRV, MCLO); else PF_WALL3_N(false, NSV, GDV, PRV, MCLO); } while (0)
#define PF_WALL3(NSV, GDV) PF_WALL3P(NSV, GDV, 0, false)
            bool profiled = false;
            if constexpr (sizeof(Real) == 4) {
               if (gi == 0 && wl_ns3 && ns == 3 && wl_geo[0] == 6 && wl_prof[0] > 0) {
                  if (wl_prof[0] == 1) PF_WALL3P(3, 6, 1, false); else PF_WALL3P(3, 6, 2, true);
                  profiled = true;
               }
            }
            if (profiled) {}
            else if (gi == 0 && wl_ns3) { if (ns == 3) { if (wl_geo[0] == 6) PF_WALL3(3, 6); else PF_WALL3(3, 0); } else if (ns == 2) PF_WALL3(2, 0); }
            else if (gi == 3 && ns == 3) {
               if constexpr (sizeof(Real) == 4) {
                  if (q == 0) {
#define PF_WALLZ3P(GDV, PRV, MCLO) do { \
                     if (mb_max <= 4 || MCLO) { if (sg) hipLaunchKernelGGL((pf::k_wall2<Real, 20, true, true, true, 4, true, 3, GDV, PRV>), gd, b, 0, st, wp, a1, a2); \
                                        else hipLaunchKernelGGL((pf::k_wall2<Real, 20, true, true, true, 4, false, 3, GDV, PRV>), gd, b, 0, st, wp, a1, a2); } \
                     else { if (sg) hipLaunchKernelGGL((pf::k_wall2<Real, 20, true, true, true, MCLO ? 4 : 12, true, 3, GDV, PRV>), gd, b, 0, st, wp, a1, a2); \
                            else hipLaunchKernelGGL((pf::k_wall2<Real, 20, true, true, true, MCLO ? 4 : 12, false, 3, GDV, PRV>), gd, b, 0, st, wp, a1, a2); } } while (0)
#define PF_WALLZ3(GDV) PF_WALLZ3P(GDV, 0, false)
                     if (wl_geo[3] == 16 && wl_prof[3] == 1) PF_WALLZ3P(16, 1, false);
                     else if (wl_geo[3] == 16 && wl_prof[3] == 2) PF_WALLZ3P(16, 2, true);
                     else if (wl_geo[3] == 16) PF_WALLZ3(16); else PF_WALLZ3(0);
#undef PF_WALLZ3P
#undef PF_WALLZ3
                  }
               }
            }
            else if (gi == 0) PF_WALL(8, false);
            else if (gi == 1) PF_WALL(12, true);
            else if (gi == 2) PF_WALL(16, true);
            else if constexpr (sizeof(Real) == 4) PF_WALL(20, true);
#undef PF_WALL3
#undef PF_WALL3P
#undef PF_WALL3_N
#undef PF_WALL
#undef PF_WALL_S
#undef PF_WALL_N
         }
      }
   }
   void launch_bricks(hipStream_t s, const Real *A, const Real *B, Real *G0, Real *G1, Real *G2, const Real *x2, const Real *x1, Real *O0, Real *O1, Real *O2, int ns) {
      if (!wl_nbrk) return;
      pf::BrickParams<Real> bp{};
      bp.x2 = x2; bp.x1 = x1;
      bp.A = A; bp.B = B; bp.G[0] = G0; bp.G[1] = G1; bp.G[2] = G2; bp.O[0] = O0; bp.O[1] = O1; bp.O[2] = O2;
      bp.plane = plane; bp.Nx = (int)Nx; bp.Ny = (int)Ny; bp.Nz = (int)Nz; bp.P = (int)P;
      bp.brk = wl_brk; bp.info = wl_binfo; bp.los = wl_blos;
      bp.sv_in = vh1; bp.sg_in = gh1; bp.sv_out = vh1b; bp.sg_out = gh1b;
      bp.ssaf = d_ssaf; bp.mat = d_mat; bp.Mb = d_Mb; bp.mq = d_mq; bp.beta = d_beta;
      bp.lo2 = lo2; bp.sl2 = sl2; bp.l = l; bp.nmat = (int)sd.Nm; bp.ns = ns;
      bp.first = op.slab_first; bp.last = op.slab_last;
      const dim3 g((unsigned)wl_nbrk), b(pf::BRICK_T);
      if (mb_max <= 4) {
         if (sg) hipLaunchKernelGGL((pf::k_brick<Real, 4, true>), g, b, wl_brk_lds, s, bp, a1, a2);
         else hipLaunchKernelGGL((pf::k_brick<Real, 4, false>), g, b, wl_brk_lds, s, bp, a1, a2);
      } else {
         if (sg) hipLaunchKernelGGL((pf::k_brick<Real, 12, true>), g, b, wl_brk_lds, s, bp, a1, a2);
         else hipLaunchKernelGGL((pf::k_brick<Real, 12, false>), g, b, wl_brk_lds, s, bp, a1, a2);
      }
   }
```

pffdtd_amd/csrc/pf_wall.h:

```cpp
#pragma once
#include <type_traits>
#include "pf_kernels.h"

namespace pf {

constexpr int WALL_MAXREG = 6;
constexpr int WALL_LT = 60;
#define PF_WALL_MAXMAT 64

struct WallRegion {
   int32_t mode;
   int32_t nbase;
   int32_t kg;
   int32_t ko0, ko1;
   int32_t kb0, kb1;
   int32_t l0, l1;
   int32_t m0, m1;
   int32_t mchunk, nlt;
   int32_t nlp;
   uint32_t blk0;
   int32_t hl, lt, hm;
   int64_t pen_off;
};

template <typename Real> struct WallParams {
   const Real *A, *B;
   Real *C, *D, *E;
   int64_t plane;
   int32_t Nx, Ny, Nz, P, first, last;
   int32_t nreg;
   WallRegion reg[WALL_MAXREG];
   const uint4 *pen;
   const uint32_t *rec;
   const uint4 *blk;
   const Real *sv_in, *sg_in;
   Real *sv_out, *sg_out;
   const Real *x2, *x1;
   Real *o1, *o2, *o3;
   const Real *ssaf;
   const int8_t *mat, *Mb;
   const MatQuadT<Real> *mq;
   const Real *beta;
   Real lo2, sl2, l;
   int32_t mmax, nmat;
};

template <typename Real, int N> __device__ __forceinline__ Real wall_sel(const Real (&a)[N], int k) {
   Real r = a[0];
#pragma unroll
   for (int i = 1; i < N; i++) {
      Real t = a[i];
      asm("" : "+v"(t));
      r = (k == i) ? t : r;
   }
   return r;
}

template <typename Real> struct WallLds {
   MatQuadT<Real> mq[PF_WALL_MAXMAT * 12];
   Real beta[PF_WALL_MAXMAT];
   int32_t M[PF_WALL_MAXMAT];
};
template <typename Real> struct WallJobs {
   Real p[64 * 8];
   int32_t li[64 * 8];
   uint32_t mask[64];
};
template <typename Real, int mmax, typename LDS = WallLds<Real>>
__device__ __forceinline__ Real fd_regs(Real p, Real u2, Real sf, int32_t k, const Real (&v1)[12], const Real (&g1)[12], Real (&v1o)[12], Real (&g1o)[12],
                                        const LDS &L, Real lo2) {
   const int M = L.M[k];
   const Real two = 2.0, one = 1.0;
   const Real g = lo2 * sf * L.beta[k];
   MatQuadT<Real> q[12];
#pragma unroll
   for (int m = 0; m < 12; m++)
      if (m < mmax) q[m] = L.mq[k * 12 + m];
   const Real fac = two * lo2 * sf / (one + g);
   Real u = p;
   u = (u + g * u2) / (one + g);
#pragma unroll
   for (int m = 0; m < 12; m++) {
      if (m < mmax) {
         const Real t = u - fac * (two * q[m].bDh * v1[m] - q[m].bFh * g1[m]);
         u = (m < M) ? t : u;
      }
   }
   const Real du = u - u2;
#pragma unroll
   for (int m = 0; m < 12; m++) {
      if (m < mmax) {
         const Real v0 = q[m].b * du + q[m].bd * v1[m] - two * q[m].bFh * g1[m];
         const Real gn = g1[m] + (v0 + v1[m]) / two;
         g1o[m] = (m < M) ? gn : g1[m];
         v1o[m] = (m < M) ? v0 : v1[m];
      } else { g1o[m] = g1[m]; v1o[m] = v1[m]; }
   }
   return u;
}

struct WallNodes { uint32_t x, z, w; };
struct WallProfileRow { int outer, inner; bool fd; };
constexpr int WALL_NPROF = 2;
constexpr WallProfileRow WALL_PROFILES[WALL_NPROF] = {{2, 3, true}, {2, 3, false}};
constexpr WallNodes wall_profile_words(int MODE, bool HI, int DP, int PR) {
   if (PR < 1 || PR > WALL_NPROF) return WallNodes{0u, 0u, 0u};
   const WallProfileRow r = WALL_PROFILES[PR - 1];
   const int ko = HI ? DP - 1 - r.outer : r.outer, ki = HI ? DP - 1 - r.inner : r.inner;
   const uint32_t all = 63u, no_p = all & ~(1u << (2 * MODE)), no_m = all & ~(2u << (2 * MODE));
   WallNodes n{(1u << ko) | (1u << ki), no_p | (no_m << 6), 0u};
   if (r.fd) n.w = (HI ? 1u : 2u) | ((uint32_t)ki << 8);
   return n;
}
template <int B, int E, typename F> __device__ __forceinline__ void wall_static_for(F &&f) {
   if constexpr (B < E) { f(std::integral_constant<int, B>()); wall_static_for<B + 1, E>(f); }
}

template <typename Real, int DP, int MODE, bool FAST, bool NODES, int MC, bool SG, int NS = 2, int GD = 0, bool HI = false, int PR = 0>
__device__ __forceinline__ void wall_body(const WallParams<Real> &wp, const WallRegion &R, const int j, const int c, const Real a1, const Real a2,
                                          const WallLds<Real> *ldsp, const uint32_t dsx, const uint32_t dsz, const uint32_t dsw, WallJobs<Real> *jobs = nullptr) {
   constexpr bool VEC = MODE == 2;
   typedef typename VecOf<Real>::type vec;
   constexpr int V = VecOf<Real>::V;
   static_assert(!VEC || DP % V == 0, "vector pencils hold whole vectors");
   const int lane = threadIdx.x;
   constexpr bool mx = MODE != 0;
   const int NL = VEC ? wp.Ny : wp.Nz;
   const int NM = mx ? wp.Nx : wp.Ny;
   const int NN = VEC ? wp.Nz : (MODE == 1 ? wp.Ny : wp.Nx);
   const bool mg_lo = mx ? (wp.first != 0) : true, mg_hi = mx ? (wp.last != 0) : true;
   const bool ng_lo = MODE == 0 ? (wp.first != 0) : true, ng_hi = MODE == 0 ? (wp.last != 0) : true;
   const int64_t sl = VEC ? (int64_t)wp.P : 1, sm = mx ? wp.plane : (int64_t)wp.P;
   const int64_t sn = VEC ? 1 : (MODE == 1 ? (int64_t)wp.P : wp.plane);
   static_assert(NS <= 2 || FAST, "three steps per pass: alike blocks only");
   const int hl = R.hl, lt = R.lt;
   const int lc = R.l0 - hl + lt * j + lane;
   int lsrc = min(max(lc, 0), NL - 1);
   if (lsrc == 0) lsrc = 2;
   else if (lsrc == NL - 1) lsrc = NL - 3;
   const bool lg_lo = lc == 0, lg_hi = lc == NL - 1;
   const bool tile_lg = !FAST && __ballot(lg_lo || lg_hi) != 0ull;
   const bool own_lane = lane >= hl && lane <= 63 - hl && lc < R.l1;
   const bool eval_lane = lane >= 1 && lane <= 62 && lc <= R.l1 + (NS == 3 ? 1 : 0);
   const int ms = R.m0 + c * R.mchunk, me = min(ms + R.mchunk, R.m1);
   if (ms >= me) return;
   const WallLds<Real> &lds = *ldsp;
   constexpr bool CG = GD > 0;
   static_assert(!CG || (FAST && NS == 3 && GD + 3 <= DP), "constant pencil geometry: alike blocks of three-step launches");
   int rkg = CG ? (HI ? DP - 1 : 0) : R.kg, rko0 = CG ? (HI ? DP - GD : 1) : R.ko0, rko1 = CG ? (HI ? DP - 1 : GD) : R.ko1;
   int rkb0 = CG ? (HI ? DP - GD - 3 : 0) : R.kb0, rkb1 = CG ? (HI ? DP : GD + 3) : R.kb1, rnbase = CG ? (HI ? NN - DP : 0) : R.nbase;
   uint32_t usx = dsx, usz = dsz, usw = dsw;
   constexpr bool PN = PR > 0;
   static_assert(!PN || (CG && NODES), "wall profiles: bodies with constant pencil geometry");
   constexpr WallNodes WN = wall_profile_words(MODE, HI, DP, PR);
   auto msrc = [&](int m) __attribute__((always_inline)) {
      m = min(max(m, 0), NM - 1);
      if (FAST) return m;
      if (m == 0 && mg_lo) return 2;
      if (m == NM - 1 && mg_hi) return NM - 3;
      return m;
   };
   const int64_t lbase = (int64_t)lsrc * sl + (int64_t)rnbase * sn;
   const int ql = (lc == 1 || lc == NL - 2) ? 1 : 0;
   const bool tile_ql = !FAST && __ballot(ql != 0) != 0ull;

   auto load_pencil = [&](const Real *G, int m, Real(&b)[DP]) __attribute__((always_inline)) {
      const Real *pl = G + (int64_t)msrc(m) * sm + lbase;
      if constexpr (VEC) {
#pragma unroll
         for (int v = 0; v < DP / V; v++) {
            const vec t = *(const vec *)(pl + v * V);
#pragma unroll
            for (int i = 0; i < V; i++) b[v * V + i] = t[i];
         }
      } else {
#pragma unroll
         for (int k = 0; k < DP; k++) b[k] = pl[(int64_t)min(max(k, rkb0), rkb1 - 1) * sn];
      }
   };
   auto mirror = [&](Real(&b)[DP]) __attribute__((always_inline)) {
#pragma unroll
      for (int k = DP - 1; k >= 0; k--) {
         const Real src = (k == 0) ? b[2] : b[k >= 2 ? k - 2 : 0];
         b[k] = (k == rkg) ? src : b[k];
      }
   };
   auto load_ent = [&](int m) __attribute__((always_inline)) {
      const uint4 *e = wp.pen + (R.pen_off + (int64_t)(min(m, R.m1 + R.hm - 1) - (R.m0 - R.hm)) * R.nlp + (lt * j + lane));
      if (FAST && (!NODES || (PN && (WN.w & 31u) == 0u))) return make_uint4(0u, 0u, 0u, 0u);
      if (FAST) return make_uint4(0u, 0u, 0u, e->w);
      return *e;
   };
   auto mask_ent = [&](uint4 e, int m) __attribute__((always_inline)) {
      if (!eval_lane || m > R.m1 + (NS == 3 ? 1 : 0)) { e.x = 0u; e.w = 0u; }
      return e;
   };
   auto store_pencil = [&](Real *G, int m, const Real(&v)[DP]) __attribute__((always_inline)) {
      if (!own_lane) return;
      Real *pl = G + (int64_t)m * sm + (int64_t)lc * sl + (int64_t)rnbase * sn;
      if constexpr (VEC) {
#pragma unroll
         for (int q = 0; q < DP / V; q++) {
            if ((q + 1) * V > rko0 && q * V < rko1) {
               vec t;
#pragma unroll
               for (int i = 0; i < V; i++) t[i] = (rkg > 0 && q * V + i > rkg) ? Real(0) : v[q * V + i];
               *(vec *)(pl + q * V) = t;
            }
         }
      } else {
#pragma unroll
         for (int k = 0; k < DP; k++)
            if (k >= rko0 && k < rko1) pl[(int64_t)k * sn] = v[k];
      }
   };
   auto fd_fetch = [&](const uint4 E, Real(&v)[12], Real(&g)[12], Real &sf, Real &u2, Real &x1v, int32_t &k) __attribute__((always_inline)) {
      if (NODES && (E.w & 31u) != 0u) {
         const int32_t li = (int32_t)(E.w >> 8);
#pragma unroll
         for (int m = 0; m < 12; m++)
            if (m < MC) { v[m] = wp.sv_in[st_idx(m, li)]; g[m] = wp.sg_in[st_idx(m, li)]; }
         sf = wp.ssaf[li];
         k = wp.mat[li];
         u2 = wp.x2[li];
         x1v = wp.x1[li];
      }
   };
   auto air = [&](Real cc, Real old, Real np_, Real nm, Real mp, Real mm, Real lp, Real lm) __attribute__((always_inline)) {
      if (MODE == 2) return upd7<SG>(a1, a2, cc, old, mp, mm, lp, lm, np_, nm);
      if (MODE == 1) return upd7<SG>(a1, a2, cc, old, mp, mm, np_, nm, lp, lm);
      return upd7<SG>(a1, a2, cc, old, np_, nm, mp, mm, lp, lm);
   };
   auto rigid = [&](uint32_t adj, Real cc, Real old, Real np_, Real nm, Real mp, Real mm, Real lp, Real lm) __attribute__((always_inline)) {
      Real nb[6];
      if (MODE == 2) { nb[0] = mp; nb[1] = mm; nb[2] = lp; nb[3] = lm; nb[4] = np_; nb[5] = nm; }
      else if (MODE == 1) { nb[0] = mp; nb[1] = mm; nb[2] = np_; nb[3] = nm; nb[4] = lp; nb[5] = lm; }
      else { nb[0] = np_; nb[1] = nm; nb[2] = mp; nb[3] = mm; nb[4] = lp; nb[5] = lm; }
      return upd_rigid<SG, 6>(a2, wp.sl2, adj, cc, old, nb);
   };

   auto update = [&](auto stage, int m, const Real(&Prv)[DP], const Real(&Cur)[DP], const Real(&Nxt)[DP], const Real(&Old)[DP], const uint4 E,
                     Real(&Out)[DP], bool own_m, const Real(&Fv)[12], const Real(&Fg)[12], Real(&Fvo)[12], Real(&Fgo)[12], Real Fsf, Real Fu2,
                     int32_t Fk, Real &nval, bool &st) __attribute__((always_inline)) {
      constexpr int STAGE = decltype(stage)::value;
      if constexpr (FAST) {
         st = false;
         if constexpr (PN) {
            constexpr uint32_t sx = WN.x, sw5 = WN.w & 31u;
            constexpr int sk0 = (int)(WN.w >> 8);
            Real pfd = Real(0);
            wall_static_for<1, DP - 1>([&](auto kc) __attribute__((always_inline)) {
               constexpr int k = decltype(kc)::value;
               const Real cc = Cur[k];
               const Real lm = lane_from_lower<true>(cc), lp = lane_from_upper<true>(cc);
               Real p;
               if constexpr (((sx >> k) & 1u) != 0u) {
                  constexpr uint32_t jn = k == 0 ? 0u : (uint32_t)__builtin_popcount(sx & ((1u << k) - 1u));
                  p = rigid((WN.z >> (6 * jn)) & 63u, cc, Old[k], Cur[k + 1], Cur[k - 1], Nxt[k], Prv[k], lp, lm);
                  if constexpr (sw5 != 0u && k == sk0) pfd = p;
               } else {
                  p = air(cc, Old[k], Cur[k + 1], Cur[k - 1], Nxt[k], Prv[k], lp, lm);
                  if constexpr (k == 1) { if (__builtin_expect(!HI && ng_lo, 0)) p = abc_loss<SG>(p, Old[k], wp.l); }
               }
               Out[k] = p;
            });
            static_assert(((sx >> 1) & 1u) == 0u && ((sx >> (DP - 2)) & 1u) == 0u, "wall profiles: no node on the ABC cell");
            if (HI && ng_hi) Out[DP - 2] = abc_loss<SG>(Out[DP - 2], Old[DP - 2], wp.l);
            if constexpr (sw5 != 0u) {
               const bool owner = own_m && own_lane && sk0 >= rko0 && sk0 < rko1;
               if (eval_lane && (STAGE < NS || STAGE == 1 || owner)) {
                  pfd = fd_regs<Real, MC>(pfd, Fu2, Fsf, Fk, Fv, Fg, Fvo, Fgo, lds, wp.lo2);
                  st = owner;
                  nval = pfd;
               }
               Out[sk0] = pfd;
            }
            mirror(Out);
            return;
         }
         const uint32_t sx = NODES ? usx : 0u, sw5 = NODES ? (usw & 31u) : 0u, sk0 = usw >> 8;
         Real pfd = Real(0);
#pragma unroll
         for (int k = 1; k < DP - 1; k++) {
            const Real cc = Cur[k];
            const Real lm = lane_from_lower<true>(cc), lp = lane_from_upper<true>(cc);
            Real p = air(cc, Old[k], Cur[k + 1], Cur[k - 1], Nxt[k], Prv[k], lp, lm);
            if (k == 1) {
               const int nk = rnbase + k;
               const bool abc1 = CG ? (!HI && ng_lo) : ((ng_lo && nk == 1) || (ng_hi && nk == NN - 2));
               if (__builtin_expect(abc1, 0)) p = abc_loss<SG>(p, Old[k], wp.l);
            }
            if (NODES && __builtin_expect(((sx >> k) & 1u) != 0u, 0)) {
               const uint32_t jn = __popc(sx & ((1u << k) - 1u));
               p = rigid((usz >> (6 * jn)) & 63u, cc, Old[k], Cur[k + 1], Cur[k - 1], Nxt[k], Prv[k], lp, lm);
               if ((uint32_t)k == sk0) pfd = p;
            }
            Out[k] = p;
         }
         if constexpr (CG) {
            if (HI && ng_hi && !(NODES && ((sx >> (DP - 2)) & 1u))) Out[DP - 2] = abc_loss<SG>(Out[DP - 2], Old[DP - 2], wp.l);
         } else {
            const int kh = NN - 2 - rnbase;
            if (ng_hi && kh >= 2 && kh <= DP - 2 && !(NODES && ((sx >> kh) & 1u))) {
               const Real t = abc_loss<SG>(wall_sel<Real, DP>(Out, kh), wall_sel<Real, DP>(Old, kh), wp.l);
#pragma unroll
               for (int k = 2; k < DP - 1; k++) Out[k] = (k == kh) ? t : Out[k];
            }
         }
         if (NODES && sw5 != 0u) {
            const bool owner = own_m && own_lane && (int)sk0 >= rko0 && (int)sk0 < rko1;
            if (eval_lane && (STAGE < NS || STAGE == 1 || owner)) {
               pfd = fd_regs<Real, MC>(pfd, Fu2, Fsf, Fk, Fv, Fg, Fvo, Fgo, lds, wp.lo2);
               st = owner;
               nval = pfd;
            }
#pragma unroll
            for (int k = 1; k < DP - 1; k++) Out[k] = ((uint32_t)k == sk0) ? pfd : Out[k];
         }
         mirror(Out);
         return;
      }
      const int qm = FAST ? 0 : (mx ? (((wp.first && m == 1) || (wp.last && m == wp.Nx - 2)) ? 1 : 0) : ((m == 1 || m == wp.Ny - 2) ? 1 : 0));
      st = false;
      const uint32_t sx = !NODES ? 0u : FAST ? usx : __builtin_amdgcn_readlane(E.x, 1), sz = FAST ? usz : __builtin_amdgcn_readlane(E.z, 1);
      const uint32_t sw5 = !NODES ? 0u : FAST ? (usw & 31u) : (__builtin_amdgcn_readlane(E.w, 1) & 31u), sk0 = FAST ? (usw >> 8) : (__builtin_amdgcn_readlane(E.y, 1) >> 27);
      bool alike = true;
      if (!FAST) {
         const bool differs = eval_lane && (E.x != sx || E.z != sz || (E.w & 31u) != sw5 || (E.y >> 27) != sk0);
         alike = __ballot(differs) == 0ull && __popc(sx) <= 5 && __popc(sw5) <= 1;
      }
      Real pfd = Real(0);
#pragma unroll
      for (int k = 1; k < DP - 1; k++) {
         const Real cc = Cur[k];
         const Real lm = lane_from_lower<true>(cc), lp = lane_from_upper<true>(cc);
         Real p = Real(0);
         const int nk = rnbase + k;
         const bool node_all = alike && ((sx >> k) & 1u);
         if (!node_all) {
            p = air(cc, Old[k], Cur[k + 1], Cur[k - 1], Nxt[k], Prv[k], lp, lm);
            const int qnm = (((ng_lo && nk == 1) || (ng_hi && nk == NN - 2)) ? 1 : 0) + qm;
            if (qnm > 0 || tile_ql) {
               const int Q = qnm + (FAST ? 0 : ql);
               if (Q > 0) p = abc_loss<SG>(p, Old[k], wp.l * (Real)Q);
            }
         }
         if (node_all) {
            const uint32_t jn = __popc(sx & ((1u << k) - 1u));
            p = rigid((sz >> (6 * jn)) & 63u, cc, Old[k], Cur[k + 1], Cur[k - 1], Nxt[k], Prv[k], lp, lm);
            if (sw5 != 0u && (uint32_t)k == sk0) pfd = p;
         }
         Out[k] = p;
      }
      if (alike) {
         if (sw5 != 0u) {
            const bool owner = own_m && own_lane && (int)sk0 >= rko0 && (int)sk0 < rko1;
            if (eval_lane && (STAGE == 1 || owner)) {
               pfd = fd_regs<Real, MC>(pfd, Fu2, Fsf, Fk, Fv, Fg, Fvo, Fgo, lds, wp.lo2);
               st = owner;
               nval = pfd;
            }
#pragma unroll
            for (int k = 1; k < DP - 1; k++)
               if ((uint32_t)k == sk0) Out[k] = pfd;
         }
      } else if (!FAST) {
         uint32_t ub = 0;
#pragma unroll
         for (int k = 1; k < DP - 1; k++)
            if (__ballot((E.x >> k) & 1u) != 0ull) ub |= 1u << k;
         const int k0 = (int)(E.y >> 27);
         uint32_t jm = 0u;
         constexpr bool BATCH = DP <= 8;
         while (ub) {
            const int k = __ffs(ub) - 1;
            ub &= ub - 1u;
            const bool has = ((E.x >> k) & 1u) != 0u;
            const int jn = __popc(E.x & ((1u << k) - 1u));
            const bool inl = jn < 5;
            const bool lossy_inl = inl && ((E.w >> jn) & 1u) != 0u;
            const bool prim = has && lossy_inl && k == k0;
            const bool need_rec = has && (!inl || (lossy_inl && !prim));
            uint32_t rec = 0u;
            if (__ballot(need_rec) != 0ull) {
               if (need_rec) rec = wp.rec[(E.y & 0x7ffffffu) + (uint32_t)jn];
            }
            const uint32_t adj = inl ? ((E.z >> (6 * jn)) & 63u) : (rec & 63u);
            const Real cc = wall_sel<Real, DP>(Cur, k), nm = wall_sel<Real, DP>(Cur, k - 1), np_ = wall_sel<Real, DP>(Cur, k + 1);
            const Real mp = wall_sel<Real, DP>(Nxt, k), mm = wall_sel<Real, DP>(Prv, k), old = wall_sel<Real, DP>(Old, k);
            const Real lm = lane_from_lower<true>(cc), lp = lane_from_upper<true>(cc);
            Real p = rigid(adj, cc, old, np_, nm, mp, mm, lp, lm);
            const bool owner = own_m && own_lane && k >= rko0 && k < rko1;
            if (prim && (STAGE == 1 || owner)) {
               p = fd_regs<Real, MC>(p, Fu2, Fsf, Fk, Fv, Fg, Fvo, Fgo, lds, wp.lo2);
               st = owner;
               nval = p;
            }
            const bool fds = has && !prim && (inl ? lossy_inl : (rec & 64u) != 0u) && (STAGE == 1 || owner);
            if (BATCH) {
               if (fds) {
                  jobs->p[lane * 8 + k] = p;
                  jobs->li[lane * 8 + k] = (int32_t)(rec >> 8) | (owner ? (1 << 30) : 0);
                  jm |= 1u << k;
               }
            } else if (__ballot(fds) != 0ull) {
               if (fds) {
                  const int32_t li = (int32_t)(rec >> 8);
                  const Real u2 = STAGE == 1 ? wp.x2[li] : wp.x1[li];
                  p = fd_core<Real>(p, u2, li, STAGE == 1 ? wp.sv_in : wp.sv_out, STAGE == 1 ? wp.sg_in : wp.sg_out, wp.sv_out, wp.sg_out, owner, wp.ssaf,
                                    wp.mat, wp.Mb, wp.mq, wp.beta, wp.lo2, wp.mmax);
                  if (owner) (STAGE == 1 ? wp.o1 : wp.o2)[li] = p;
               }
            }
#pragma unroll
            for (int i = 1; i < DP - 1; i++) Out[i] = (has && k == i) ? p : Out[i];
         }
         if (BATCH && __ballot(jm != 0u) != 0ull) {
            jobs->mask[lane] = jm;
            __syncthreads();
            for (int t = 0; t < 8; t++) {
               const int slot = t * 64 + lane, src = slot >> 3, kk = slot & 7;
               const bool valid = ((jobs->mask[src] >> kk) & 1u) != 0u;
               if (__ballot(valid) != 0ull) {
                  if (valid) {
                     const int32_t w = jobs->li[slot], li = w & 0x3fffffff;
                     const bool own = (w >> 30) != 0;
                     const Real u2 = STAGE == 1 ? wp.x2[li] : wp.x1[li];
                     const Real r = fd_core<Real>(jobs->p[slot], u2, li, STAGE == 1 ? wp.sv_in : wp.sv_out, STAGE == 1 ? wp.sg_in : wp.sg_out, wp.sv_out, wp.sg_out, own,
                                                  wp.ssaf, wp.mat, wp.Mb, wp.mq, wp.beta, wp.lo2, wp.mmax);
                     if (own) (STAGE == 1 ? wp.o1 : wp.o2)[li] = r;
                     jobs->p[slot] = r;
                  }
               }
            }
            __syncthreads();
#pragma unroll
            for (int i = 1; i < DP - 1; i++)
               if ((jm >> i) & 1u) Out[i] = jobs->p[lane * 8 + i];
            __syncthreads();
         }
      }
      mirror(Out);
      if (STAGE == 1 && tile_lg) {
#pragma unroll
         for (int k = 0; k < DP; k++) {
            const Real t = Out[k];
            const Real up = __shfl(t, lane + 2, 64), dn = __shfl(t, lane - 2, 64);
            Out[k] = lg_lo ? up : (lg_hi ? dn : t);
         }
      }
   };

   Real Bm[DP], Bc[DP], Bn[DP], Bq[DP], Ac[DP], Aq[DP], Vm[DP], Vc[DP], Vn[DP], W[DP];
   Real Xm[NS == 3 ? DP : 1], Xc[NS == 3 ? DP : 1], Y[NS == 3 ? DP : 1];
   Real F1v[12], F1g[12], Fqv[12], Fqg[12], F2v[12], F2g[12];
   Real F3v[NS == 3 ? 12 : 1], F3g[NS == 3 ? 12 : 1];
   Real F1sf = 0, F1u2 = 0, F1x1 = 0, Fqsf = 0, Fqu2 = 0, Fqx1 = 0, F2sf = 0, F2u2 = 0, F3sf = 0, F3u2 = 0, F2n1 = 0;
   int32_t F1k = 0, Fqk = 0, F2k = 0, F3k = 0;
#pragma unroll
   for (int q = 0; q < 12; q++) { F1v[q] = F1g[q] = Fqv[q] = Fqg[q] = F2v[q] = F2g[q] = Real(0); if (NS == 3) F3v[q] = F3g[q] = Real(0); }
   const int mf = NS == 1 ? ms : ms - (NS - 1), ml = NS == 1 ? me - 1 : me + (NS - 2);
   uint4 Epp = make_uint4(0u, 0u, 0u, 0u), Ep = make_uint4(0u, 0u, 0u, 0u), Ec = mask_ent(load_ent(mf), mf), En = mask_ent(load_ent(mf + 1), mf + 1), Eq;
   load_pencil(wp.B, mf - 1, Bm);
   load_pencil(wp.B, mf, Bc);
   load_pencil(wp.B, mf + 1, Bn);
   load_pencil(wp.A, mf, Ac);
   mirror(Bm); mirror(Bc); mirror(Bn);
   fd_fetch(Ec, F1v, F1g, F1sf, F1u2, F1x1, F1k);
#pragma unroll
   for (int k = 0; k < DP; k++) { Vm[k] = Real(0); Vc[k] = Real(0); Vn[k] = Real(0); W[k] = Real(0); }
   if constexpr (NS == 3) {
#pragma unroll
      for (int k = 0; k < DP; k++) { Xm[k] = Real(0); Xc[k] = Real(0); Y[k] = Real(0); }
   }
   Eq = load_ent(mf + 2);
   load_pencil(wp.B, mf + 2, Bq);
   load_pencil(wp.A, mf + 1, Aq);
   fd_fetch(En, Fqv, Fqg, Fqsf, Fqu2, Fqx1, Fqk);
   for (int m = mf; m <= ml; m++) {
      usx = dsx; usz = dsz; usw = dsw;
      if constexpr (PN) {}
      else if constexpr (CG) asm volatile("" : "+s"(usx), "+s"(usz), "+s"(usw));
      else {
         rkg = R.kg; rko0 = R.ko0; rko1 = R.ko1; rkb0 = R.kb0; rkb1 = R.kb1; rnbase = R.nbase;
         asm volatile("" : "+s"(rkg), "+s"(rko0), "+s"(rko1), "+s"(rkb0), "+s"(rkb1), "+s"(rnbase), "+s"(usx), "+s"(usz), "+s"(usw));
      }
      const bool own_m = m >= ms && m < me;
      Real nv1 = Real(0), nv2 = Real(0), nv3 = Real(0);
      bool st1 = false, st2 = false, st3 = false;
      update(std::integral_constant<int, 1>(), m, Bm, Bc, Bn, Ac, Ec, Vn, own_m, F1v, F1g, F1v, F1g, F1sf, F1u2, F1k, nv1, st1);
      if constexpr (PN) {}
      else if constexpr (CG) asm volatile("" : "+s"(usx), "+s"(usz), "+s"(usw));
      else asm volatile("" : "+s"(rkg), "+s"(rko0), "+s"(rko1), "+s"(rnbase), "+s"(usx), "+s"(usz), "+s"(usw));
      const bool do2 = NS >= 2 && m - 1 >= ms - (NS - 2);
      const bool own_m2 = m - 1 >= ms && m - 1 < me;
      if (do2) {
         if (!mx && !FAST) {
            const bool sub_hi = m == NM - 1 && mg_hi, sub_lo = m - 2 == 0 && mg_lo;
            Real Pv[DP], Nv[DP];
#pragma unroll
            for (int k = 0; k < DP; k++) { Pv[k] = sub_lo ? Vn[k] : Vm[k]; Nv[k] = sub_hi ? Vm[k] : Vn[k]; }
            update(std::integral_constant<int, 2>(), m - 1, Pv, Vc, Nv, Bm, Ep, W, true, F2v, F2g, F2v, F2g, F2sf, F2u2, F2k, nv2, st2);
         } else update(std::integral_constant<int, 2>(), m - 1, Vm, Vc, Vn, Bm, Ep, W, own_m2, F2v, F2g, F2v, F2g, F2sf, F2u2, F2k, nv2, st2);
      }
      const bool do3 = NS == 3 && m - 2 >= ms;
      if constexpr (NS == 3) {
         if constexpr (PN) {}
         else if constexpr (CG) asm volatile("" : "+s"(usx), "+s"(usz), "+s"(usw));
         else asm volatile("" : "+s"(rkg), "+s"(rko0), "+s"(rko1), "+s"(rnbase), "+s"(usx), "+s"(usz), "+s"(usw));
         if (do3) update(std::integral_constant<int, 3>(), m - 2, Xm, Xc, W, Vm, Epp, Y, true, F3v, F3g, F3v, F3g, F3sf, F3u2, F3k, nv3, st3);
      }
      const int32_t li1 = (int32_t)(Ec.w >> 8), li2 = (int32_t)(Ep.w >> 8), li3 = (int32_t)(Epp.w >> 8);
#pragma unroll
      for (int k = 0; k < DP; k++) { Vm[k] = Vc[k]; Vc[k] = Vn[k]; Bm[k] = Bc[k]; Bc[k] = Bn[k]; Bn[k] = Bq[k]; Ac[k] = Aq[k]; }
#pragma unroll
      for (int k = 0; k < DP; k++) { asm volatile("" : "+v"(Bn[k])); asm volatile("" : "+v"(Ac[k])); }
#pragma unroll
      for (int q = 0; q < 12; q++) { asm volatile("" : "+v"(Fqv[q])); asm volatile("" : "+v"(Fqg[q])); }
      asm volatile("" : "+v"(Fqsf), "+v"(Fqu2), "+v"(Fqx1), "+v"(Fqk), "+v"(Eq.x), "+v"(Eq.y), "+v"(Eq.z), "+v"(Eq.w) : : "memory");
      mirror(Bn);
      if (own_m) store_pencil(wp.C, m, Vc);
      if (do2 && own_m2) store_pencil(wp.D, m - 1, W);
      if constexpr (NS == 3) { if (do3) store_pencil(wp.E, m - 2, Y); }
      if (st1) wp.o1[li1] = nv1;
      if (NS == 1 && st1) {
#pragma unroll
         for (int q = 0; q < 12; q++)
            if (q < MC) { wp.sv_out[st_idx(q, li1)] = F1v[q]; wp.sg_out[st_idx(q, li1)] = F1g[q]; }
      }
      if (st2) {
         wp.o2[li2] = nv2;
         if (NS == 2) {
#pragma unroll
            for (int q = 0; q < 12; q++)
               if (q < MC) { wp.sv_out[st_idx(q, li2)] = F2v[q]; wp.sg_out[st_idx(q, li2)] = F2g[q]; }
         }
      }
      if constexpr (NS == 3) {
         if (st3) {
            wp.o3[li3] = nv3;
#pragma unroll
            for (int q = 0; q < 12; q++)
               if (q < MC) { wp.sv_out[st_idx(q, li3)] = F3v[q]; wp.sg_out[st_idx(q, li3)] = F3g[q]; }
         }
      }
      asm volatile("" : : : "memory");
      if constexpr (NS == 3) {
#pragma unroll
         for (int k = 0; k < DP; k++) { Xm[k] = Xc[k]; Xc[k] = W[k]; }
#pragma unroll
         for (int q = 0; q < 12; q++) { F3v[q] = F2v[q]; F3g[q] = F2g[q]; }
         F3sf = F2sf; F3k = F2k; F3u2 = F2n1;
         F2n1 = nv1;
      }
#pragma unroll
      for (int q = 0; q < 12; q++) { F2v[q] = F1v[q]; F2g[q] = F1g[q]; F1v[q] = Fqv[q]; F1g[q] = Fqg[q]; }
      F2sf = F1sf; F2u2 = F1x1; F2k = F1k;
      F1sf = Fqsf; F1u2 = Fqu2; F1x1 = Fqx1; F1k = Fqk;
      Epp = Ep; Ep = Ec; Ec = En; En = mask_ent(Eq, m + 2);
      if (m + 1 <= ml) {
         Eq = load_ent(m + 3);
         if (m + 1 < ml) {
            load_pencil(wp.B, m + 3, Bq);
            load_pencil(wp.A, m + 2, Aq);
            fd_fetch(En, Fqv, Fqg, Fqsf, Fqu2, Fqx1, Fqk);
         }
      }
   }
}

template <typename Real, int DP, bool VEC, bool FAST, bool NODES = true, int MC = 12, bool SG = false, int NS = 2, int GD = 0, int PR = 0>
__global__ __launch_bounds__(64) __attribute__((amdgpu_waves_per_eu((FAST && !VEC && NS != 3 && sizeof(Real) == 4) ? 2 : 1))) void k_wall2(WallParams<Real> wp, Real a1, Real a2) {
   static_assert(FAST || NODES, "generic blocks have everything");
   const uint4 bd = wp.blk[blockIdx.x];
   const WallRegion R = wp.reg[bd.x & 7u];
   const int j = (int)((bd.x >> 3) & 0x1fffu), c = (int)(bd.x >> 16);
   __shared__ WallLds<Real> lds;
   __shared__ typename std::conditional<FAST, int, WallJobs<Real>>::type jobs_mem;
   WallJobs<Real> *jobs = nullptr;
   if constexpr (!FAST) {
      jobs = &jobs_mem;
      jobs->mask[threadIdx.x] = 0u;
   }
   if (NODES) {
      for (int i = threadIdx.x; i < wp.nmat * 12; i += 64) lds.mq[i] = wp.mq[i];
      for (int i = threadIdx.x; i < wp.nmat; i += 64) { lds.beta[i] = wp.beta[i]; lds.M[i] = wp.Mb[i]; }
      __syncthreads();
   }
   static_assert(PR == 0 || GD > 0, "wall profiles: with constant pencil geometry");
   if constexpr (GD > 0) {
      const bool hi = R.kg != 0;
      if constexpr (VEC) { if (hi) wall_body<Real, DP, 2, FAST, NODES, MC, SG, NS, GD, true, PR>(wp, R, j, c, a1, a2, &lds, bd.y, bd.z, bd.w, jobs);
                           else wall_body<Real, DP, 2, FAST, NODES, MC, SG, NS, GD, false, PR>(wp, R, j, c, a1, a2, &lds, bd.y, bd.z, bd.w, jobs); }
      else if (R.mode == 1) { if (hi) wall_body<Real, DP, 1, FAST, NODES, MC, SG, NS, GD, true, PR>(wp, R, j, c, a1, a2, &lds, bd.y, bd.z, bd.w, jobs);
                              else wall_body<Real, DP, 1, FAST, NODES, MC, SG, NS, GD, false, PR>(wp, R, j, c, a1, a2, &lds, bd.y, bd.z, bd.w, jobs); }
      else { if (hi) wall_body<Real, DP, 0, FAST, NODES, MC, SG, NS, GD, true, PR>(wp, R, j, c, a1, a2, &lds, bd.y, bd.z, bd.w, jobs);
             else wall_body<Real, DP, 0, FAST, NODES, MC, SG, NS, GD, false, PR>(wp, R, j, c, a1, a2, &lds, bd.y, bd.z, bd.w, jobs); }
   } else if constexpr (VEC) wall_body<Real, DP, 2, FAST, NODES, MC, SG, NS>(wp, R, j, c, a1, a2, &lds, bd.y, bd.z, bd.w, jobs);
   else if (R.mode == 1) wall_body<Real, DP, 1, FAST, NODES, MC, SG, NS>(wp, R, j, c, a1, a2, &lds, bd.y, bd.z, bd.w, jobs);
   else wall_body<Real, DP, 0, FAST, NODES, MC, SG, NS>(wp, R, j, c, a1, a2, &lds, bd.y, bd.z, bd.w, jobs);
}

}
```

pffdtd_amd/engine.py:

```python
import ctypes
import importlib.util
import os
import sys
from pathlib import Path

import numpy as np

from .sim_data import PfSimData

_HERE = Path(__file__).resolve().parent
_LIB = None

PF_NUM_CPU_EXACT = 0
PF_NUM_GPU_SAFEGUARDED = 2


class PfOpts(ctypes.Structure):
    _fields_ = [("device", ctypes.c_int32), ("numerics", ctypes.c_int32), ("slab_first", ctypes.c_int32),
                ("slab_last", ctypes.c_int32), ("readout_chunk", ctypes.c_int32), ("air_variant", ctypes.c_int32),
                ("air_chunk", ctypes.c_int32), ("timing", ctypes.c_int32), ("ext_u0", ctypes.c_void_p),
                ("ext_u1", ctypes.c_void_p), ("x_global0", ctypes.c_int32), ("layout", ctypes.c_int32),
                ("energy", ctypes.c_int32), ("multi_flags", ctypes.c_int32), ("transport", ctypes.c_int32),
                ("verify_exchange", ctypes.c_int32), ("only_slab", ctypes.c_int32), ("wall_scale", ctypes.c_double)]


_HOOKS = ("debug", "test_drop_exchange", "test_faults")


def _set_hooks(debug=0, test_drop_exchange=0, test_faults=0):
    lib().pf_internal_hooks(int(debug), int(test_drop_exchange), int(test_faults))


class PfTiming(ctypes.Structure):
    _fields_ = [("air_ms_total", ctypes.c_double), ("air_launches", ctypes.c_int64),
                ("step_ms_total", ctypes.c_double), ("steps", ctypes.c_int64),
                ("tb2_ms_total", ctypes.c_double), ("tb2_launches", ctypes.c_int64), ("tb2_cells", ctypes.c_int64),
                ("tune_ms", ctypes.c_double * 3), ("air_path", ctypes.c_int64), ("tb2_lw", ctypes.c_int64),
                ("tb2_dirty_tiles", ctypes.c_int64), ("place_candidates", ctypes.c_int64), ("place_ms", ctypes.c_double * 3),
                ("wall_blocks", ctypes.c_int64 * 2), ("tb_steps_per_pass", ctypes.c_int64), ("wall_bricks", ctypes.c_int64), ("wall_three_steps", ctypes.c_int64),
                ("wall_profile", ctypes.c_int64)]


class PfMultiInfo(ctypes.Structure):
    _fields_ = [("nslabs", ctypes.c_int32), ("transport", ctypes.c_int32), ("rccl_self", ctypes.c_int32),
                ("exchange_verified", ctypes.c_int32), ("exchanges_checked", ctypes.c_int64),
                ("exchange_nonzero", ctypes.c_int32), ("cut_along_z", ctypes.c_int32), ("plane_bytes", ctypes.c_int64),
                ("last_run_seconds", ctypes.c_double), ("transport_name", ctypes.c_char * 64),
                ("transport_note", ctypes.c_char * 256), ("wall_scale", ctypes.c_double), ("wall_measured", ctypes.c_int32)]


class PfError(RuntimeError):
    pass


EXPORTS = ["pf_last_error", "pf_version", "pf_device_count", "pf_grid_bytes", "pf_grid_pitch", "pf_opts_default",
           "pf_run_sim", "pf_engine_create", "pf_engine_destroy", "pf_engine_run", "pf_engine_step_begin",
           "pf_engine_halo_ptrs", "pf_engine_step_end", "pf_engine_state_grids", "pf_engine_layout", "pf_engine_place_grids", "pf_engine_place_grids5", "pf_engine_set_spares", "pf_engine_stream", "pf_engine_sync",
           "pf_engine_flush_outputs", "pf_engine_get_grid", "pf_engine_set_grid", "pf_engine_timing", "pf_engine_set_timing",
           "pf_engine_energy_cfg", "pf_engine_run_energy", "pf_run_sim_devices", "pf_slab_partition", "pf_slab_partition_w", "pf_slab_partition_axis", "pf_slab_wall_scale",
           "pf_multi_create", "pf_multi_run", "pf_multi_get_info", "pf_multi_get_slab", "pf_multi_destroy",
           "pf_rccl_unique_id", "pf_rccl_comm_create", "pf_rccl_exchange", "pf_rccl_comm_destroy"]


INTERNAL_EXPORTS = ["pf_internal_hooks"]

PF_MULTI_EVEN_SPLIT, PF_MULTI_ONE_THREAD, PF_MULTI_NO_PAIRS, PF_MULTI_FORCE_PAIRS, PF_MULTI_CUT_Z, PF_MULTI_CUT_X = 1, 2, 4, 8, 16, 32
PF_MULTI_NO_TRIPLES = 64
PF_MULTI_MEASURE_WEIGHTS = 128
PF_TRANSPORT_AUTO, PF_TRANSPORT_PEER, PF_TRANSPORT_RCCL, PF_TRANSPORT_HOST = 0, 1, 2, 3
PF_LAYOUT_AUTO, PF_LAYOUT_EXCHANGED, PF_LAYOUT_FILE = 0, 1, 2


def _preload_torch_hip():
    if "torch" in sys.modules or os.environ.get("PFFDTD_SYSTEM_HIP") == "1":
        return
    try:
        spec = importlib.util.find_spec("torch")
    except (ImportError, ValueError):
        return
    if spec is None or not spec.submodule_search_locations:
        return
    p = Path(spec.submodule_search_locations[0]) / "lib" / "libamdhip64.so"
    if p.exists():
        try:
            ctypes.CDLL(str(p), mode=ctypes.RTLD_GLOBAL)
        except OSError:
            pass


def lib_path():
    return _HERE / "libpffdtd_hip.so"


def lib():
    global _LIB
    if _LIB is None:
        p = lib_path()
        if not p.exists():
            raise PfError(f"{p} not built: run `python -c 'import __graft_entry__ as g; g.build()'`")
        _preload_torch_hip()
        L = ctypes.CDLL(str(p))
        vp, i32, i64 = ctypes.c_void_p, ctypes.c_int32, ctypes.c_int64
        L.pf_last_error.restype = ctypes.c_char_p
        L.pf_version.restype = ctypes.c_char_p
        L.pf_device_count.restype = ctypes.c_int
        L.pf_grid_bytes.restype = ctypes.c_size_t
        L.pf_grid_bytes.argtypes = [i64, i64, i64, i32]
        L.pf_grid_pitch.restype = i64
        L.pf_grid_pitch.argtypes = [i64, i32]
        L.pf_opts_default.argtypes = [ctypes.POINTER(PfOpts)]
        L.pf_internal_hooks.argtypes = [ctypes.c_int32, ctypes.c_int32, ctypes.c_int32]
        L.pf_internal_hooks.restype = None
        L.pf_run_sim.restype = ctypes.c_double
        L.pf_run_sim.argtypes = [ctypes.POINTER(PfSimData)]
        L.pf_engine_create.argtypes = [ctypes.POINTER(PfSimData), ctypes.POINTER(PfOpts), ctypes.POINTER(vp)]
        L.pf_engine_destroy.argtypes = [vp]
        L.pf_engine_destroy.restype = None
        L.pf_engine_run.argtypes = [vp, i64, i64]
        L.pf_engine_step_begin.argtypes = [vp, i64]
        L.pf_engine_step_end.argtypes = [vp, i64]
        L.pf_engine_halo_ptrs.argtypes = [vp, ctypes.POINTER(vp), ctypes.POINTER(vp), ctypes.POINTER(vp),
                                          ctypes.POINTER(vp), ctypes.POINTER(ctypes.c_size_t)]
        L.pf_engine_state_grids.argtypes = [vp, ctypes.POINTER(vp), ctypes.POINTER(vp)]
        L.pf_engine_layout.argtypes = [vp, ctypes.POINTER(i64), ctypes.POINTER(i64), ctypes.POINTER(i32)]
        L.pf_engine_place_grids.argtypes = [vp, ctypes.POINTER(vp), i32, ctypes.POINTER(i32)]
        L.pf_engine_place_grids5.argtypes = [vp, ctypes.POINTER(vp), i32, ctypes.POINTER(i32)]
        L.pf_engine_stream.restype = vp
        L.pf_engine_stream.argtypes = [vp, i32]
        L.pf_engine_sync.argtypes = [vp]
        L.pf_engine_flush_outputs.argtypes = [vp]
        L.pf_engine_get_grid.argtypes = [vp, i32, vp]
        L.pf_engine_set_grid.argtypes = [vp, i32, vp]
        L.pf_engine_timing.argtypes = [vp, ctypes.POINTER(PfTiming), i32]
        L.pf_engine_set_timing.argtypes = [vp, i32]
        dp = ctypes.POINTER(ctypes.c_double)
        L.pf_engine_energy_cfg.argtypes = [vp, ctypes.c_double, ctypes.c_double, ctypes.c_double, dp]
        L.pf_engine_run_energy.argtypes = [vp, i64, i64, dp, dp, dp]
        L.pf_run_sim_devices.restype = ctypes.c_double
        L.pf_run_sim_devices.argtypes = [ctypes.POINTER(PfSimData), i32, ctypes.POINTER(i32), ctypes.POINTER(PfOpts)]
        L.pf_slab_partition.argtypes = [ctypes.POINTER(PfSimData), i32, i32, ctypes.POINTER(i64)]
        L.pf_slab_partition_w.argtypes = [ctypes.POINTER(PfSimData), i32, i32, ctypes.c_double, ctypes.POINTER(i64)]
        L.pf_slab_partition_axis.argtypes = [ctypes.POINTER(PfSimData), i32, i32, ctypes.c_double, i32, ctypes.POINTER(i64)]
        L.pf_slab_wall_scale.argtypes = [ctypes.POINTER(PfSimData), i32, i32, ctypes.POINTER(PfOpts)]
        L.pf_slab_wall_scale.restype = ctypes.c_double
        L.pf_engine_set_spares.argtypes = [vp, vp, vp]
        L.pf_multi_create.argtypes = [ctypes.POINTER(PfSimData), i32, ctypes.POINTER(i32), ctypes.POINTER(PfOpts), ctypes.POINTER(vp)]
        L.pf_multi_run.argtypes = [vp, i64, i64]
        L.pf_multi_get_info.argtypes = [vp, ctypes.POINTER(PfMultiInfo)]
        L.pf_multi_get_slab.argtypes = [vp, i32, ctypes.POINTER(i64), ctypes.POINTER(i64), ctypes.POINTER(i32), ctypes.POINTER(i32), ctypes.POINTER(vp)]
        L.pf_multi_destroy.argtypes = [vp]
        L.pf_multi_destroy.restype = None
        L.pf_rccl_unique_id.argtypes = [ctypes.c_char_p]
        L.pf_rccl_comm_create.argtypes = [ctypes.c_char_p, i32, i32, i32, ctypes.POINTER(ctypes.c_void_p)]
        L.pf_rccl_exchange.argtypes = [ctypes.c_void_p, ctypes.c_void_p, i32, i32]
        L.pf_rccl_comm_destroy.argtypes = [ctypes.c_void_p]
        L.pf_rccl_comm_destroy.restype = None
        _LIB = L
    return _LIB


def _check(rc):
    if rc != 0:
        raise PfError(f"pffdtd_hip error {rc}: {lib().pf_last_error().decode()}")


def device_count():
    return int(lib().pf_device_count())


def grid_pitch(Nz, real_bytes):
    return int(lib().pf_grid_pitch(int(Nz), int(real_bytes)))


def run_sim(sd):
    s = sd.as_struct()
    el = lib().pf_run_sim(ctypes.byref(s))
    if el < 0:
        raise PfError(f"pf_run_sim failed: {lib().pf_last_error().decode()}")
    return el


def run_sim_devices(sd, devices, multi_flags=0, **opts):
    L = lib()
    s = sd.as_struct()
    o = _multi_opts(multi_flags, opts)
    devs = (ctypes.c_int32 * len(devices))(*[int(d) for d in devices])
    el = L.pf_run_sim_devices(ctypes.byref(s), len(devices), devs, ctypes.byref(o))
    if el < 0:
        raise PfError(f"pf_run_sim_devices failed: {L.pf_last_error().decode()}")
    return el


def _multi_opts(multi_flags, opts):
    o = PfOpts()
    lib().pf_opts_default(ctypes.byref(o))
    hooks = {k: opts[k] for k in _HOOKS if k in opts}
    for k, v in opts.items():
        if k not in _HOOKS:
            setattr(o, k, float(v) if k == "wall_scale" else int(v))
    o.multi_flags = int(multi_flags)
    _set_hooks(**hooks)
    return o


class HipMulti:

    def __init__(self, sd, devices, multi_flags=0, **opts):
        L = lib()
        self.sd = sd
        self._s = sd.as_struct()
        o = _multi_opts(multi_flags, opts)
        devs = (ctypes.c_int32 * len(devices))(*[int(d) for d in devices])
        self._h = ctypes.c_void_p()
        _check(L.pf_multi_create(ctypes.byref(self._s), len(devices), devs, ctypes.byref(o), ctypes.byref(self._h)))
        self.nslabs = len(devices)

    def run(self, n0, nsteps):
        _check(lib().pf_multi_run(self._h, int(n0), int(nsteps)))

    def info(self):
        i = PfMultiInfo()
        _check(lib().pf_multi_get_info(self._h, ctypes.byref(i)))
        return {"nslabs": i.nslabs, "transport": i.transport, "transport_name": i.transport_name.decode(),
                "rccl_self": bool(i.rccl_self), "exchanges_checked": i.exchanges_checked,
                "exchange_verified": None if i.exchange_verified < 0 else bool(i.exchange_verified),
                "exchange_nonzero": bool(i.exchange_nonzero), "cut_along_z": bool(i.cut_along_z), "plane_bytes": i.plane_bytes,
                "last_run_seconds": i.last_run_seconds, "transport_note": i.transport_note.decode(),
                "wall_scale": i.wall_scale, "wall_measured": bool(i.wall_measured)}

    def slab(self, g):
        x0, x1, dev, pr, eh = ctypes.c_int64(), ctypes.c_int64(), ctypes.c_int32(), ctypes.c_int32(), ctypes.c_void_p()
        _check(lib().pf_multi_get_slab(self._h, int(g), ctypes.byref(x0), ctypes.byref(x1), ctypes.byref(dev), ctypes.byref(pr), ctypes.byref(eh)))
        spp = {0: 0, 1: 2, 3: 3}.get(int(pr.value), 2)
        return {"x0": x0.value, "x1": x1.value, "device": dev.value, "paired": spp > 0, "steps_per_pass": spp, "engine": _EngineView(eh, self.sd.real_bytes)}

    def close(self):
        if getattr(self, "_h", None) and self._h.value:
            lib().pf_multi_destroy(self._h)
            self._h = ctypes.c_void_p()

    def __del__(self):
        try:
            self.close()
        except Exception:
            pass


class _EngineView:

    def __init__(self, handle, real_bytes):
        self._h = handle
        self.dtype = np.float32 if real_bytes == 4 else np.float64

    state_grids = lambda self: HipEngine.state_grids(self)
    layout = lambda self: HipEngine.layout(self)
    timing = lambda self, reset=False: HipEngine.timing(self, reset)
    sync = lambda self: HipEngine.sync(self)
    set_timing = lambda self, on: HipEngine.set_timing(self, on)


def slab_partition(sd, nslabs, even=False, wall_scale=1.0, along_z=False):
    s = sd.as_struct()
    cuts = (ctypes.c_int64 * (nslabs + 1))()
    _check(lib().pf_slab_partition_axis(ctypes.byref(s), int(nslabs), int(bool(even)), float(wall_scale), int(bool(along_z)), cuts))
    return [(int(cuts[g]), int(cuts[g + 1])) for g in range(nslabs)]


def slab_wall_scale(sd, nslabs, device=0, **opts):
    s = sd.as_struct()
    o = _multi_opts(0, opts)
    k = float(lib().pf_slab_wall_scale(ctypes.byref(s), int(nslabs), int(device), ctypes.byref(o)))
    return k if k > 0 else None


class HipEngine:

    def __init__(self, sd, device=0, numerics=PF_NUM_CPU_EXACT, slab_first=True, slab_last=True, air_variant=0,
                 air_chunk=0, timing=False, readout_chunk=0, ext_u0=None, ext_u1=None, debug=0, x_global0=0, energy=False, layout=0):
        L = lib()
        self.sd = sd
        self._s = sd.as_struct()
        o = PfOpts()
        L.pf_opts_default(ctypes.byref(o))
        o.device, o.numerics = int(device), int(numerics)
        o.slab_first, o.slab_last = int(bool(slab_first)), int(bool(slab_last))
        o.air_variant, o.air_chunk, o.timing, o.readout_chunk = int(air_variant), int(air_chunk), int(bool(timing)), \
            int(readout_chunk)
        o.x_global0 = int(x_global0)
        o.layout = int(layout)
        o.energy = int(bool(energy))
        if ext_u0 is not None and ext_u1 is not None:
            o.ext_u0, o.ext_u1 = int(ext_u0), int(ext_u1)
        self._h = ctypes.c_void_p()
        _set_hooks(debug=debug)
        _check(L.pf_engine_create(ctypes.byref(self._s), ctypes.byref(o), ctypes.byref(self._h)))
        self.dtype = np.float32 if sd.real_bytes == 4 else np.float64

    def run(self, n0, nsteps):
        _check(lib().pf_engine_run(self._h, int(n0), int(nsteps)))

    def step_begin(self, n):
        _check(lib().pf_engine_step_begin(self._h, int(n)))

    def step_end(self, n):
        _check(lib().pf_engine_step_end(self._h, int(n)))

    def halo_ptrs(self):
        vp = ctypes.c_void_p
        slo, shi, rlo, rhi, nb = vp(), vp(), vp(), vp(), ctypes.c_size_t()
        _check(lib().pf_engine_halo_ptrs(self._h, ctypes.byref(slo), ctypes.byref(shi), ctypes.byref(rlo),
                                         ctypes.byref(rhi), ctypes.byref(nb)))
        return slo.value, shi.value, rlo.value, rhi.value, nb.value

    def state_grids(self):
        vp = ctypes.c_void_p
        up, uc = vp(), vp()
        _check(lib().pf_engine_state_grids(self._h, ctypes.byref(up), ctypes.byref(uc)))
        return up.value, uc.value

    def layout(self):
        dims, pitch, ex = (ctypes.c_int64 * 3)(), ctypes.c_int64(), ctypes.c_int32()
        _check(lib().pf_engine_layout(self._h, dims, ctypes.byref(pitch), ctypes.byref(ex)))
        return (int(dims[0]), int(dims[1]), int(dims[2])), int(pitch.value), bool(ex.value)

    def place_grids(self, ptrs):
        arr = (ctypes.c_void_p * len(ptrs))(*[int(p) for p in ptrs])
        idx = (ctypes.c_int32 * 4)()
        _check(lib().pf_engine_place_grids(self._h, arr, len(ptrs), idx))
        return idx[2] >= 0, list(idx)

    def place_grids5(self, ptrs):
        arr = (ctypes.c_void_p * len(ptrs))(*[int(p) for p in ptrs])
        idx = (ctypes.c_int32 * 5)()
        _check(lib().pf_engine_place_grids5(self._h, arr, len(ptrs), idx))
        return (3 if idx[4] >= 0 else (2 if idx[2] >= 0 else 0)), list(idx)

    def set_spares(self, ptr2, ptr3):
        rc = lib().pf_engine_set_spares(self._h, ctypes.c_void_p(ptr2), ctypes.c_void_p(ptr3))
        if rc not in (0, 1):
            _check(rc)
        return rc == 0

    def stream(self, which):
        return lib().pf_engine_stream(self._h, int(which))

    def sync(self):
        _check(lib().pf_engine_sync(self._h))

    def flush_outputs(self):
        _check(lib().pf_engine_flush_outputs(self._h))

    def get_grid(self, which):
        a = np.empty((self.sd.Nx, self.sd.Ny, self.sd.Nz), dtype=self.dtype)
        _check(lib().pf_engine_get_grid(self._h, int(which), a.ctypes.data_as(ctypes.c_void_p)))
        return a

    def set_grid(self, which, a):
        a = np.ascontiguousarray(a, dtype=self.dtype)
        assert a.size == self.sd.Npts
        _check(lib().pf_engine_set_grid(self._h, int(which), a.ctypes.data_as(ctypes.c_void_p)))

    def energy_cfg(self, h, c, Ts, DEF_list):
        tab = np.zeros((max(len(DEF_list), 1), 12, 3), dtype=np.float64)
        for k, d in enumerate(DEF_list):
            tab[k, :d.shape[0]] = d
        self._DEF = tab
        dp = ctypes.POINTER(ctypes.c_double)
        _check(lib().pf_engine_energy_cfg(self._h, float(h), float(c), float(Ts), tab.ctypes.data_as(dp)))

    def run_energy(self, n0, nsteps, H_tot, E_lost, E_in):
        dp = ctypes.POINTER(ctypes.c_double)
        for a in (H_tot, E_lost, E_in):
            assert a.dtype == np.float64 and a.flags["C_CONTIGUOUS"]
        _check(lib().pf_engine_run_energy(self._h, int(n0), int(nsteps), H_tot.ctypes.data_as(dp),
                                          E_lost.ctypes.data_as(dp), E_in.ctypes.data_as(dp)))

    def timing(self, reset=False):
        t = PfTiming()
        _check(lib().pf_engine_timing(self._h, ctypes.byref(t), int(reset)))
        return {"air_ms_total": t.air_ms_total, "air_launches": t.air_launches, "step_ms_total": t.step_ms_total,
                "steps": t.steps, "tb2_ms_total": t.tb2_ms_total, "tb2_launches": t.tb2_launches, "tb2_cells": t.tb2_cells,
                "tune_ms": list(t.tune_ms), "air_path": t.air_path, "tb2_lw": t.tb2_lw, "tb2_dirty_tiles": t.tb2_dirty_tiles,
                "place_candidates": t.place_candidates, "place_ms": list(t.place_ms), "wall_blocks": list(t.wall_blocks),
                "tb_steps_per_pass": t.tb_steps_per_pass, "wall_bricks": t.wall_bricks, "wall_three_steps": t.wall_three_steps, "wall_profile": t.wall_profile}

    def set_timing(self, on):
        _check(lib().pf_engine_set_timing(self._h, int(bool(on))))

    def close(self):
        if getattr(self, "_h", None) and self._h.value:
            lib().pf_engine_destroy(self._h)
            self._h = ctypes.c_void_p()

    def __del__(self):
        try:
            self.close()
        except Exception:
            pass
```

Before: 831.8 Gvoxel-updates/s.

## Specialize three-step wall kernels for uniform branch counts and skip unread first-step stores

When every material has the same number of frequency-dependent branches (e.g. 11), new wall kernel variants use that count as a compile-time constant. This drops the per-branch M selects and moves only the live branch state. Coefficients are pre-scaled into a row-major LDS layout so they can be loaded as vectors. When no receiver, dirty tile or leftover list reads the first-step pencil output, that store is skipped, which removes global writes at the cost of extra conditions tying correctness to readout placement.

After: 844.9 Gvoxel-updates/s, median of 6. +1.6%, better.

```diff
diff --git a/include/pffdtd_hip.h b/include/pffdtd_hip.h
--- a/include/pffdtd_hip.h
+++ b/include/pffdtd_hip.h
@@ -111,6 +111,8 @@
    int64_t wall_bricks;
    int64_t wall_three_steps;
    int64_t wall_profile;
+   int64_t wall_uniform_branches;
+   int64_t wall_unread_skipped;
 } pf_timing;
 
 typedef struct pf_engine pf_engine;
diff --git a/pffdtd_amd/csrc/pf_debug.h b/pffdtd_amd/csrc/pf_debug.h
--- a/pffdtd_amd/csrc/pf_debug.h
+++ b/pffdtd_amd/csrc/pf_debug.h
@@ -9,6 +9,8 @@
 pf_opts_x pf__take_hooks(const pf_opts *o);
 int pf__engine_create_x(const pf_simdata *sd, const pf_opts_x *o, pf_engine **out);
 enum : int {
+   PF_DBG_BRANCH_SELECTS = 0x1,
+   PF_DBG_STORE_UNREAD = 0x2,
    PF_DBG_RUNTIME_NODES = 0x20,
    PF_DBG_LW32 = 0x100,
    PF_DBG_LW16 = 0x200,
diff --git a/pffdtd_amd/csrc/pf_engine_class.inc b/pffdtd_amd/csrc/pf_engine_class.inc
--- a/pffdtd_amd/csrc/pf_engine_class.inc
+++ b/pffdtd_amd/csrc/pf_engine_class.inc
@@ -220,6 +220,15 @@
    Real *ubx[2] = {nullptr, nullptr};
    int wl_geo[4] = {0, 0, 0, 0};
    int wl_prof[4] = {0, 0, 0, 0};
+   int wl_uni = 0;
+   unsigned wl_rcv = 0;
+   bool wl_uni_group(int gi) const {
+      return sizeof(Real) == 4 && wl_uni > 0 && wl_prof[gi] == 1 && ((gi == 0 && wl_ns3 && wl_geo[0] == 6) || (gi == 3 && wl_ns3z && wl_geo[3] == 16));
+   }
+   bool wl_skip_c(int gi) const {
+      return wl_uni_group(gi) && op.slab_first && op.slab_last && tb_ndirty == 0 && wl_nrest == 0 && !((wl_rcv >> gi) & 1u) &&
+             !(op.debug & (PF_DBG_STORE_UNREAD | PF_DBG_THIRD_STEP_LISTS));
+   }
    int wl_chunk_want[2] = {0, 0};
    size_t wl_brk_lds = 0;
    Real *vh1b = nullptr, *gh1b = nullptr;
@@ -823,6 +832,9 @@
       tm.wall_bricks = wl_on ? wl_nbrk : 0;
       tm.wall_three_steps = (wl_on && (tb3 || (tb3_slab && ws_all3))) ? ((wl_ns3 ? 1 : 0) | (wl_ns3z ? 8 : 0) | (wl_xw[0] ? 0x10 : 0) | (wl_xw[1] ? 0x20 : 0)) : 0;
       tm.wall_profile = (((tm.wall_three_steps & 1) && wl_geo[0] == 6 && wl_prof[0]) ? 1 : 0) | (((tm.wall_three_steps & 8) && wl_geo[3] == 16 && wl_prof[3]) ? 8 : 0);
+      tm.wall_uniform_branches = 0; tm.wall_unread_skipped = 0;
+      for (int gi : {0, 3})
+         if (((tm.wall_profile >> gi) & 1) && wl_uni_group(gi)) { tm.wall_uniform_branches = wl_uni; if (wl_skip_c(gi)) tm.wall_unread_skipped |= (int64_t)1 << gi; }
       if (t) *t = tm;
       if (reset) tm = pf_timing{};
       return PF_OK;
diff --git a/pffdtd_amd/csrc/pf_engine_walls.inc b/pffdtd_amd/csrc/pf_engine_walls.inc
--- a/pffdtd_amd/csrc/pf_engine_walls.inc
+++ b/pffdtd_amd/csrc/pf_engine_walls.inc
@@ -16,7 +16,7 @@
    void free_walls() {
       auto F = [](auto *&p) { if (p) hipFree((void *)p); p = nullptr; };
       F(wl_pen); F(wl_rec); F(wl_rest); F(wl_blk); F(wl_brk); F(wl_binfo); F(wl_blos); F(vh1b); F(gh1b); F(ubx[0]); F(ubx[1]);
-      wl_nbrk = 0; wl_brk_lds = 0; wl_ns3 = wl_ns3z = false;
+      wl_nbrk = 0; wl_brk_lds = 0; wl_ns3 = wl_ns3z = false; wl_uni = 0; wl_rcv = 0;
       for (int &p : wl_prof) p = 0;
       wl_xw[0] = wl_xw[1] = false;
       wl_on = false;
@@ -430,6 +430,22 @@
             if (all) wl_prof[gi] = pr;
          }
       }
+      wl_uni = 0;
+      {
+         bool uni = sd.Nm > 0 && !(op.debug & PF_DBG_BRANCH_SELECTS);
+         for (int k = 0; k < sd.Nm; k++) uni = uni && sd.Mb[k] == mb_max;
+         if (uni && (mb_max == 11 || mb_max == 12 || (mb_max >= 1 && mb_max <= 4))) wl_uni = mb_max;
+      }
+      wl_rcv = 0;
+      for (int64_t i = 0; i < Nr; i++) {
+         int64_t ix, iy, iz;
+         decode(sd.out_ixyz[i], ix, iy, iz);
+         for (int r = 0; r < nregs; r++) {
+            int k, lc, m;
+            frame(reg[r], ix, iy, iz, k, lc, m);
+            if (k >= reg[r].ko0 && k < reg[r].ko1 && lc >= reg[r].l0 && lc < reg[r].l1 && m >= reg[r].m0 && m < reg[r].m1) wl_rcv |= 1u << grp[r];
+         }
+      }
       wl_ns3 = ns3; wl_ns3z = ns3z;
       if ((ns3 && wl_grp[0].nblk[1] > 0) || (ns3z && wl_grp[3].nblk[1] > 0)) {
          wl_no_ns3 = true;
@@ -460,6 +476,8 @@
          const WlGroup &g = wl_grp[gi];
          wp.nreg = g.nreg;
          for (int i = 0; i < g.nreg; i++) wp.reg[i] = g.reg[i];
+         const bool uni = ns == 3 && wl_uni_group(gi);
+         wp.C = (uni && wl_skip_c(gi)) ? nullptr : C;
          for (int q = 0; q < 3; q++) {
             if (!g.nblk[q]) continue;
             wp.blk = wl_blk + g.blk0[q];
@@ -483,10 +501,16 @@
                               else hipLaunchKernelGGL((pf::k_wall2<Real, 10, false, true, true, MCLO ? 4 : 12, S, NSV, GDV, PRV>), gd, b, 0, st, wp, a1, a2); } while (0)
 #define PF_WALL3P(NSV, GDV, PRV, MCLO) do { if (sg) PF_WALL3_N(true, NSV, GDV, PRV, MCLO); else PF_WALL3_N(false, NSV, GDV, PRV, MCLO); } while (0)
 #define PF_WALL3(NSV, GDV) PF_WALL3P(NSV, GDV, 0, false)
+#define PF_WALLU(DPV, VECV, GDV, MCV, UBV, USKV) do { if (q != 0) break; \
+                              if (sg) hipLaunchKernelGGL((pf::k_wall2<Real, DPV, VECV, true, true, MCV, true, 3, GDV, 1, UBV, USKV>), gd, b, 0, st, wp, a1, a2); \
+                              else hipLaunchKernelGGL((pf::k_wall2<Real, DPV, VECV, true, true, MCV, false, 3, GDV, 1, UBV, USKV>), gd, b, 0, st, wp, a1, a2); } while (0)
+#define PF_WALLU_ANY(DPV, VECV, GDV) do { if (wl_uni == 11) PF_WALLU(DPV, VECV, GDV, 12, 11, false); else if (wl_uni == 12) PF_WALLU(DPV, VECV, GDV, 12, 12, false); \
+                              else PF_WALLU(DPV, VECV, GDV, 4, 4, true); } while (0)
             bool profiled = false;
             if constexpr (sizeof(Real) == 4) {
                if (gi == 0 && wl_ns3 && ns == 3 && wl_geo[0] == 6 && wl_prof[0] > 0) {
-                  if (wl_prof[0] == 1) PF_WALL3P(3, 6, 1, false); else PF_WALL3P(3, 6, 2, true);
+                  if (uni) PF_WALLU_ANY(10, false, 6);
+                  else if (wl_prof[0] == 1) PF_WALL3P(3, 6, 1, false); else PF_WALL3P(3, 6, 2, true);
                   profiled = true;
                }
             }
@@ -501,7 +525,8 @@
                      else { if (sg) hipLaunchKernelGGL((pf::k_wall2<Real, 20, true, true, true, MCLO ? 4 : 12, true, 3, GDV, PRV>), gd, b, 0, st, wp, a1, a2); \
                             else hipLaunchKernelGGL((pf::k_wall2<Real, 20, true, true, true, MCLO ? 4 : 12, false, 3, GDV, PRV>), gd, b, 0, st, wp, a1, a2); } } while (0)
 #define PF_WALLZ3(GDV) PF_WALLZ3P(GDV, 0, false)
-                     if (wl_geo[3] == 16 && wl_prof[3] == 1) PF_WALLZ3P(16, 1, false);
+                     if (uni) PF_WALLU_ANY(20, true, 16);
+                     else if (wl_geo[3] == 16 && wl_prof[3] == 1) PF_WALLZ3P(16, 1, false);
                      else if (wl_geo[3] == 16 && wl_prof[3] == 2) PF_WALLZ3P(16, 2, true);
                      else if (wl_geo[3] == 16) PF_WALLZ3(16); else PF_WALLZ3(0);
 #undef PF_WALLZ3P
@@ -513,6 +538,8 @@
             else if (gi == 1) PF_WALL(12, true);
             else if (gi == 2) PF_WALL(16, true);
             else if constexpr (sizeof(Real) == 4) PF_WALL(20, true);
+#undef PF_WALLU_ANY
+#undef PF_WALLU
 #undef PF_WALL3
 #undef PF_WALL3P
 #undef PF_WALL3_N
diff --git a/pffdtd_amd/csrc/pf_wall.h b/pffdtd_amd/csrc/pf_wall.h
--- a/pffdtd_amd/csrc/pf_wall.h
+++ b/pffdtd_amd/csrc/pf_wall.h
@@ -66,37 +66,87 @@
    int32_t li[64 * 8];
    uint32_t mask[64];
 };
-template <typename Real, int mmax, typename LDS = WallLds<Real>>
+constexpr int WALL_UROWS = 5, WALL_UROW = 12;
+template <typename Real> struct WallLdsU {
+   alignas(16) Real c[PF_WALL_MAXMAT][WALL_UROWS * WALL_UROW];
+   Real beta[PF_WALL_MAXMAT];
+   template <typename Q> __device__ __forceinline__ void put(int i, const Q &q) {
+      const Real two = 2.0;
+      Real *r = c[i / 12] + i % 12;
+      r[0] = two * q.bDh; r[WALL_UROW] = q.bFh; r[2 * WALL_UROW] = q.b; r[3 * WALL_UROW] = q.bd; r[4 * WALL_UROW] = two * q.bFh;
+   }
+};
+template <typename Real, int mmax, typename LDS = WallLds<Real>, int MB = mmax, bool UNI = false, bool SKIP = false>
 __device__ __forceinline__ Real fd_regs(Real p, Real u2, Real sf, int32_t k, const Real (&v1)[12], const Real (&g1)[12], Real (&v1o)[12], Real (&g1o)[12],
-                                        const LDS &L, Real lo2) {
-   const int M = L.M[k];
-   const Real two = 2.0, one = 1.0;
-   const Real g = lo2 * sf * L.beta[k];
-   MatQuadT<Real> q[12];
-#pragma unroll
-   for (int m = 0; m < 12; m++)
-      if (m < mmax) q[m] = L.mq[k * 12 + m];
-   const Real fac = two * lo2 * sf / (one + g);
-   Real u = p;
-   u = (u + g * u2) / (one + g);
-#pragma unroll
-   for (int m = 0; m < 12; m++) {
-      if (m < mmax) {
-         const Real t = u - fac * (two * q[m].bDh * v1[m] - q[m].bFh * g1[m]);
-         u = (m < M) ? t : u;
-      }
+                                        const LDS &L, Real lo2, int nb = MB) {
+   if constexpr (UNI) {
+      static_assert(MB >= 1 && MB <= mmax && mmax <= WALL_UROW, "uniform branch count within the state the kernel moves");
+      typedef typename VecOf<Real>::type vec;
+      constexpr int V = VecOf<Real>::V, NV = (MB + V - 1) / V;
+      const Real two = 2.0, one = 1.0;
+      const Real g = lo2 * sf * L.beta[k];
+      Real cf[WALL_UROWS][NV * V];
+      auto rows = [&](int32_t kk, int r0, int r1) __attribute__((always_inline)) {
+         const vec *cp = (const vec *)L.c[kk];
+#pragma unroll
+         for (int r = r0; r < r1; r++)
+#pragma unroll
+            for (int v = 0; v < NV; v++) {
+               const vec t = cp[r * (WALL_UROW / V) + v];
+#pragma unroll
+               for (int i = 0; i < V; i++) cf[r][v * V + i] = t[i];
+            }
+      };
+      rows(k, 0, 2);
+      const Real fac = two * lo2 * sf / (one + g);
+      Real u = p;
+      u = (u + g * u2) / (one + g);
+#pragma unroll
+      for (int m = 0; m < MB; m++)
+         if (!SKIP || m < nb) u = u - fac * (cf[0][m] * v1[m] - cf[1][m] * g1[m]);
+      const Real du = u - u2;
+      int32_t k2 = k;
+      asm("" : "+v"(k2) : "v"(du));
+      rows(k2, 2, WALL_UROWS);
+#pragma unroll
+      for (int m = 0; m < MB; m++) {
+         if (!SKIP || m < nb) {
+            const Real v0 = cf[2][m] * du + cf[3][m] * v1[m] - cf[4][m] * g1[m];
+            g1o[m] = g1[m] + (v0 + v1[m]) / two;
+            v1o[m] = v0;
+         } else { g1o[m] = g1[m]; v1o[m] = v1[m]; }
+      }
+      return u;
+   } else {
+      const int M = L.M[k];
+      const Real two = 2.0, one = 1.0;
+      const Real g = lo2 * sf * L.beta[k];
+      MatQuadT<Real> q[12];
+#pragma unroll
+      for (int m = 0; m < 12; m++)
+         if (m < mmax) q[m] = L.mq[k * 12 + m];
+      const Real fac = two * lo2 * sf / (one + g);
+      Real u = p;
+      u = (u + g * u2) / (one + g);
+#pragma unroll
+      for (int m = 0; m < 12; m++) {
+         if (m < mmax) {
+            const Real t = u - fac * (two * q[m].bDh * v1[m] - q[m].bFh * g1[m]);
+            u = (m < M) ? t : u;
+         }
+      }
+      const Real du = u - u2;
+#pragma unroll
+      for (int m = 0; m < 12; m++) {
+         if (m < mmax) {
+            const Real v0 = q[m].b * du + q[m].bd * v1[m] - two * q[m].bFh * g1[m];
+            const Real gn = g1[m] + (v0 + v1[m]) / two;
+            g1o[m] = (m < M) ? gn : g1[m];
+            v1o[m] = (m < M) ? v0 : v1[m];
+         } else { g1o[m] = g1[m]; v1o[m] = v1[m]; }
+      }
+      return u;
    }
-   const Real du = u - u2;
-#pragma unroll
-   for (int m = 0; m < 12; m++) {
-      if (m < mmax) {
-         const Real v0 = q[m].b * du + q[m].bd * v1[m] - two * q[m].bFh * g1[m];
-         const Real gn = g1[m] + (v0 + v1[m]) / two;
-         g1o[m] = (m < M) ? gn : g1[m];
-         v1o[m] = (m < M) ? v0 : v1[m];
-      } else { g1o[m] = g1[m]; v1o[m] = v1[m]; }
-   }
-   return u;
 }
 
 struct WallNodes { uint32_t x, z, w; };
@@ -116,9 +166,10 @@
    if constexpr (B < E) { f(std::integral_constant<int, B>()); wall_static_for<B + 1, E>(f); }
 }
 
-template <typename Real, int DP, int MODE, bool FAST, bool NODES, int MC, bool SG, int NS = 2, int GD = 0, bool HI = false, int PR = 0>
+template <typename Real, int DP, int MODE, bool FAST, bool NODES, int MC, bool SG, int NS = 2, int GD = 0, bool HI = false, int PR = 0, int UB = 0, bool USK = false,
+          typename LDS = WallLds<Real>>
 __device__ __forceinline__ void wall_body(const WallParams<Real> &wp, const WallRegion &R, const int j, const int c, const Real a1, const Real a2,
-                                          const WallLds<Real> *ldsp, const uint32_t dsx, const uint32_t dsz, const uint32_t dsw, WallJobs<Real> *jobs = nullptr) {
+                                          const LDS *ldsp, const uint32_t dsx, const uint32_t dsz, const uint32_t dsw, WallJobs<Real> *jobs = nullptr) {
    constexpr bool VEC = MODE == 2;
    typedef typename VecOf<Real>::type vec;
    constexpr int V = VecOf<Real>::V;
@@ -144,7 +195,9 @@
    const bool eval_lane = lane >= 1 && lane <= 62 && lc <= R.l1 + (NS == 3 ? 1 : 0);
    const int ms = R.m0 + c * R.mchunk, me = min(ms + R.mchunk, R.m1);
    if (ms >= me) return;
-   const WallLds<Real> &lds = *ldsp;
+   const LDS &lds = *ldsp;
+   constexpr int NB = UB > 0 ? UB : MC, NQ = UB > 0 ? UB : 12;
+   static_assert(UB == 0 || (PR > 0 && NS == 3 && UB <= MC), "uniform branch counts: profiled three-step bodies");
    constexpr bool CG = GD > 0;
    static_assert(!CG || (FAST && NS == 3 && GD + 3 <= DP), "constant pencil geometry: alike blocks of three-step launches");
    int rkg = CG ? (HI ? DP - 1 : 0) : R.kg, rko0 = CG ? (HI ? DP - GD : 1) : R.ko0, rko1 = CG ? (HI ? DP - 1 : GD) : R.ko1;
@@ -219,7 +272,7 @@
          const int32_t li = (int32_t)(E.w >> 8);
 #pragma unroll
          for (int m = 0; m < 12; m++)
-            if (m < MC) { v[m] = wp.sv_in[st_idx(m, li)]; g[m] = wp.sg_in[st_idx(m, li)]; }
+            if (m < NB) { v[m] = wp.sv_in[st_idx(m, li)]; g[m] = wp.sg_in[st_idx(m, li)]; }
          sf = wp.ssaf[li];
          k = wp.mat[li];
          u2 = wp.x2[li];
@@ -269,7 +322,8 @@
             if constexpr (sw5 != 0u) {
                const bool owner = own_m && own_lane && sk0 >= rko0 && sk0 < rko1;
                if (eval_lane && (STAGE < NS || STAGE == 1 || owner)) {
-                  pfd = fd_regs<Real, MC>(pfd, Fu2, Fsf, Fk, Fv, Fg, Fvo, Fgo, lds, wp.lo2);
+                  if constexpr (UB > 0) pfd = fd_regs<Real, MC, LDS, UB, true, USK>(pfd, Fu2, Fsf, Fk, Fv, Fg, Fvo, Fgo, lds, wp.lo2, USK ? wp.mmax : UB);
+                  else pfd = fd_regs<Real, MC>(pfd, Fu2, Fsf, Fk, Fv, Fg, Fvo, Fgo, lds, wp.lo2);
                   st = owner;
                   nval = pfd;
                }
@@ -310,7 +364,7 @@
          if (NODES && sw5 != 0u) {
             const bool owner = own_m && own_lane && (int)sk0 >= rko0 && (int)sk0 < rko1;
             if (eval_lane && (STAGE < NS || STAGE == 1 || owner)) {
-               pfd = fd_regs<Real, MC>(pfd, Fu2, Fsf, Fk, Fv, Fg, Fvo, Fgo, lds, wp.lo2);
+               if constexpr (UB == 0) pfd = fd_regs<Real, MC>(pfd, Fu2, Fsf, Fk, Fv, Fg, Fvo, Fgo, lds, wp.lo2);
                st = owner;
                nval = pfd;
             }
@@ -356,7 +410,7 @@
          if (sw5 != 0u) {
             const bool owner = own_m && own_lane && (int)sk0 >= rko0 && (int)sk0 < rko1;
             if (eval_lane && (STAGE == 1 || owner)) {
-               pfd = fd_regs<Real, MC>(pfd, Fu2, Fsf, Fk, Fv, Fg, Fvo, Fgo, lds, wp.lo2);
+               if constexpr (UB == 0) pfd = fd_regs<Real, MC>(pfd, Fu2, Fsf, Fk, Fv, Fg, Fvo, Fgo, lds, wp.lo2);
                st = owner;
                nval = pfd;
             }
@@ -392,7 +446,7 @@
             Real p = rigid(adj, cc, old, np_, nm, mp, mm, lp, lm);
             const bool owner = own_m && own_lane && k >= rko0 && k < rko1;
             if (prim && (STAGE == 1 || owner)) {
-               p = fd_regs<Real, MC>(p, Fu2, Fsf, Fk, Fv, Fg, Fvo, Fgo, lds, wp.lo2);
+               if constexpr (UB == 0) p = fd_regs<Real, MC>(p, Fu2, Fsf, Fk, Fv, Fg, Fvo, Fgo, lds, wp.lo2);
                st = owner;
                nval = p;
             }
@@ -516,10 +570,11 @@
 #pragma unroll
       for (int k = 0; k < DP; k++) { asm volatile("" : "+v"(Bn[k])); asm volatile("" : "+v"(Ac[k])); }
 #pragma unroll
-      for (int q = 0; q < 12; q++) { asm volatile("" : "+v"(Fqv[q])); asm volatile("" : "+v"(Fqg[q])); }
+      for (int q = 0; q < NQ; q++) { asm volatile("" : "+v"(Fqv[q])); asm volatile("" : "+v"(Fqg[q])); }
       asm volatile("" : "+v"(Fqsf), "+v"(Fqu2), "+v"(Fqx1), "+v"(Fqk), "+v"(Eq.x), "+v"(Eq.y), "+v"(Eq.z), "+v"(Eq.w) : : "memory");
       mirror(Bn);
-      if (own_m) store_pencil(wp.C, m, Vc);
+      if constexpr (UB > 0) { if (own_m && wp.C) store_pencil(wp.C, m, Vc); }
+      else if (own_m) store_pencil(wp.C, m, Vc);
       if (do2 && own_m2) store_pencil(wp.D, m - 1, W);
       if constexpr (NS == 3) { if (do3) store_pencil(wp.E, m - 2, Y); }
       if (st1) wp.o1[li1] = nv1;
@@ -541,7 +596,7 @@
             wp.o3[li3] = nv3;
 #pragma unroll
             for (int q = 0; q < 12; q++)
-               if (q < MC) { wp.sv_out[st_idx(q, li3)] = F3v[q]; wp.sg_out[st_idx(q, li3)] = F3g[q]; }
+               if (q < NB) { wp.sv_out[st_idx(q, li3)] = F3v[q]; wp.sg_out[st_idx(q, li3)] = F3g[q]; }
          }
       }
       asm volatile("" : : : "memory");
@@ -549,12 +604,12 @@
 #pragma unroll
          for (int k = 0; k < DP; k++) { Xm[k] = Xc[k]; Xc[k] = W[k]; }
 #pragma unroll
-         for (int q = 0; q < 12; q++) { F3v[q] = F2v[q]; F3g[q] = F2g[q]; }
+         for (int q = 0; q < NQ; q++) { F3v[q] = F2v[q]; F3g[q] = F2g[q]; }
          F3sf = F2sf; F3k = F2k; F3u2 = F2n1;
          F2n1 = nv1;
       }
 #pragma unroll
-      for (int q = 0; q < 12; q++) { F2v[q] = F1v[q]; F2g[q] = F1g[q]; F1v[q] = Fqv[q]; F1g[q] = Fqg[q]; }
+      for (int q = 0; q < NQ; q++) { F2v[q] = F1v[q]; F2g[q] = F1g[q]; F1v[q] = Fqv[q]; F1g[q] = Fqg[q]; }
       F2sf = F1sf; F2u2 = F1x1; F2k = F1k;
       F1sf = Fqsf; F1u2 = Fqu2; F1x1 = Fqx1; F1k = Fqk;
       Epp = Ep; Ep = Ec; Ec = En; En = mask_ent(Eq, m + 2);
@@ -569,20 +624,25 @@
    }
 }
 
-template <typename Real, int DP, bool VEC, bool FAST, bool NODES = true, int MC = 12, bool SG = false, int NS = 2, int GD = 0, int PR = 0>
+template <typename Real, int DP, bool VEC, bool FAST, bool NODES = true, int MC = 12, bool SG = false, int NS = 2, int GD = 0, int PR = 0, int UB = 0, bool USK = false>
 __global__ __launch_bounds__(64) __attribute__((amdgpu_waves_per_eu((FAST && !VEC && NS != 3 && sizeof(Real) == 4) ? 2 : 1))) void k_wall2(WallParams<Real> wp, Real a1, Real a2) {
    static_assert(FAST || NODES, "generic blocks have everything");
    const uint4 bd = wp.blk[blockIdx.x];
    const WallRegion R = wp.reg[bd.x & 7u];
    const int j = (int)((bd.x >> 3) & 0x1fffu), c = (int)(bd.x >> 16);
-   __shared__ WallLds<Real> lds;
+   typedef typename std::conditional<(UB > 0), WallLdsU<Real>, WallLds<Real>>::type LDS;
+   __shared__ LDS lds;
    __shared__ typename std::conditional<FAST, int, WallJobs<Real>>::type jobs_mem;
    WallJobs<Real> *jobs = nullptr;
    if constexpr (!FAST) {
       jobs = &jobs_mem;
       jobs->mask[threadIdx.x] = 0u;
    }
-   if (NODES) {
+   if constexpr (UB > 0) {
+      for (int i = threadIdx.x; i < wp.nmat * 12; i += 64) lds.put(i, wp.mq[i]);
+      for (int i = threadIdx.x; i < wp.nmat; i += 64) lds.beta[i] = wp.beta[i];
+      __syncthreads();
+   } else if (NODES) {
       for (int i = threadIdx.x; i < wp.nmat * 12; i += 64) lds.mq[i] = wp.mq[i];
       for (int i = threadIdx.x; i < wp.nmat; i += 64) { lds.beta[i] = wp.beta[i]; lds.M[i] = wp.Mb[i]; }
       __syncthreads();
@@ -590,12 +650,12 @@
    static_assert(PR == 0 || GD > 0, "wall profiles: with constant pencil geometry");
    if constexpr (GD > 0) {
       const bool hi = R.kg != 0;
-      if constexpr (VEC) { if (hi) wall_body<Real, DP, 2, FAST, NODES, MC, SG, NS, GD, true, PR>(wp, R, j, c, a1, a2, &lds, bd.y, bd.z, bd.w, jobs);
-                           else wall_body<Real, DP, 2, FAST, NODES, MC, SG, NS, GD, false, PR>(wp, R, j, c, a1, a2, &lds, bd.y, bd.z, bd.w, jobs); }
-      else if (R.mode == 1) { if (hi) wall_body<Real, DP, 1, FAST, NODES, MC, SG, NS, GD, true, PR>(wp, R, j, c, a1, a2, &lds, bd.y, bd.z, bd.w, jobs);
-                              else wall_body<Real, DP, 1, FAST, NODES, MC, SG, NS, GD, false, PR>(wp, R, j, c, a1, a2, &lds, bd.y, bd.z, bd.w, jobs); }
-      else { if (hi) wall_body<Real, DP, 0, FAST, NODES, MC, SG, NS, GD, true, PR>(wp, R, j, c, a1, a2, &lds, bd.y, bd.z, bd.w, jobs);
-             else wall_body<Real, DP, 0, FAST, NODES, MC, SG, NS, GD, false, PR>(wp, R, j, c, a1, a2, &lds, bd.y, bd.z, bd.w, jobs); }
+      if constexpr (VEC) { if (hi) wall_body<Real, DP, 2, FAST, NODES, MC, SG, NS, GD, true, PR, UB, USK, LDS>(wp, R, j, c, a1, a2, &lds, bd.y, bd.z, bd.w, jobs);
+                           else wall_body<Real, DP, 2, FAST, NODES, MC, SG, NS, GD, false, PR, UB, USK, LDS>(wp, R, j, c, a1, a2, &lds, bd.y, bd.z, bd.w, jobs); }
+      else if (R.mode == 1) { if (hi) wall_body<Real, DP, 1, FAST, NODES, MC, SG, NS, GD, true, PR, UB, USK, LDS>(wp, R, j, c, a1, a2, &lds, bd.y, bd.z, bd.w, jobs);
+                              else wall_body<Real, DP, 1, FAST, NODES, MC, SG, NS, GD, false, PR, UB, USK, LDS>(wp, R, j, c, a1, a2, &lds, bd.y, bd.z, bd.w, jobs); }
+      else { if (hi) wall_body<Real, DP, 0, FAST, NODES, MC, SG, NS, GD, true, PR, UB, USK, LDS>(wp, R, j, c, a1, a2, &lds, bd.y, bd.z, bd.w, jobs);
+             else wall_body<Real, DP, 0, FAST, NODES, MC, SG, NS, GD, false, PR, UB, USK, LDS>(wp, R, j, c, a1, a2, &lds, bd.y, bd.z, bd.w, jobs); }
    } else if constexpr (VEC) wall_body<Real, DP, 2, FAST, NODES, MC, SG, NS>(wp, R, j, c, a1, a2, &lds, bd.y, bd.z, bd.w, jobs);
    else if (R.mode == 1) wall_body<Real, DP, 1, FAST, NODES, MC, SG, NS>(wp, R, j, c, a1, a2, &lds, bd.y, bd.z, bd.w, jobs);
    else wall_body<Real, DP, 0, FAST, NODES, MC, SG, NS>(wp, R, j, c, a1, a2, &lds, bd.y, bd.z, bd.w, jobs);
diff --git a/pffdtd_amd/engine.py b/pffdtd_amd/engine.py
--- a/pffdtd_amd/engine.py
+++ b/pffdtd_amd/engine.py
@@ -38,7 +38,7 @@
                 ("tune_ms", ctypes.c_double * 3), ("air_path", ctypes.c_int64), ("tb2_lw", ctypes.c_int64),
                 ("tb2_dirty_tiles", ctypes.c_int64), ("place_candidates", ctypes.c_int64), ("place_ms", ctypes.c_double * 3),
                 ("wall_blocks", ctypes.c_int64 * 2), ("tb_steps_per_pass", ctypes.c_int64), ("wall_bricks", ctypes.c_int64), ("wall_three_steps", ctypes.c_int64),
-                ("wall_profile", ctypes.c_int64)]
+                ("wall_profile", ctypes.c_int64), ("wall_uniform_branches", ctypes.c_int64), ("wall_unread_skipped", ctypes.c_int64)]
 
 
 class PfMultiInfo(ctypes.Structure):
@@ -382,7 +382,8 @@
                 "steps": t.steps, "tb2_ms_total": t.tb2_ms_total, "tb2_launches": t.tb2_launches, "tb2_cells": t.tb2_cells,
                 "tune_ms": list(t.tune_ms), "air_path": t.air_path, "tb2_lw": t.tb2_lw, "tb2_dirty_tiles": t.tb2_dirty_tiles,
                 "place_candidates": t.place_candidates, "place_ms": list(t.place_ms), "wall_blocks": list(t.wall_blocks),
-                "tb_steps_per_pass": t.tb_steps_per_pass, "wall_bricks": t.wall_bricks, "wall_three_steps": t.wall_three_steps, "wall_profile": t.wall_profile}
+                "tb_steps_per_pass": t.tb_steps_per_pass, "wall_bricks": t.wall_bricks, "wall_three_steps": t.wall_three_steps, "wall_profile": t.wall_profile,
+                "wall_uniform_branches": t.wall_uniform_branches, "wall_unread_skipped": t.wall_unread_skipped}
 
     def set_timing(self, on):
         _check(lib().pf_engine_set_timing(self._h, int(bool(on))))
```
